# stevenrobertson/cuburn

Hardware: AMD Instinct MI355X
Metric: Msamples/s into 1920x1080 histogram + DE-filter GB/s vs HBM roofline (higher is better)
Workload: dtype f32; 1 GPU; BASELINE configs[1]: 1920x1080 still, 3 xforms (linear+spherical+swirl), 2^28 samples/frame, filters yuv+bilateral+logscale+colorclip, rgba8 out; walker_waves=4, walker_slots=1024, temporal_samples=1024, samples_per_frame=268435456, accum=binned, fuse=256, nslots=1024, frames_queued_ahead=2, frames_per_gpu=1121, parallelism=frame-sharded x1, RCCL gather of device frames, 4 frames per collective

## Files before the change

cuburn_amd/csrc/de.hip:

```cpp
#include "flame_device.h"
#include "kernels.h"
#include "tone_device.h"
#include <utility>
#include <cmath>
#include <algorithm>
#include <cstdlib>
#include <cstring>

struct DeImgPlain {
    float4 *p;
    __device__ __forceinline__ float4 ld(uint32_t i) const { return const_cast<const float4 *>(p)[i]; }
    __device__ __forceinline__ void st(uint32_t i, float4 v) const { p[i] = v; }
};
struct DeCoefs { float k[7]; float k2[19]; };
struct DeSpatial { float s[16]; };

__host__ __device__ constexpr int de_num_x(int P) { constexpr int n[8] = {2, 0, 2, -2, 2, -1, 2, 1}; return n[P]; }
__host__ __device__ constexpr int de_num_y(int P) { constexpr int n[8] = {0, 2, 2, 2, 1, 2, -1, 2}; return n[P]; }
__host__ __device__ constexpr int de_rne_half(int v)
{
    return (v % 2 == 0) ? v / 2 : ((v - 1) / 2 % 2 == 0 ? (v - 1) / 2 : (v + 1) / 2);
}
__host__ __device__ constexpr int de_dx(int P, int r) { return de_rne_half(de_num_x(P) * r); }
__host__ __device__ constexpr int de_dy(int P, int r) { return de_rne_half(de_num_y(P) * r); }
__host__ __device__ constexpr int de_k(int P) { constexpr int k[8] = {0, 0, 2, -2, 4, -1, -4, 1}; return k[P]; }
__host__ __device__ constexpr int de_floor_half(int v) { return v >= 0 ? v / 2 : -((-v + 1) / 2); }
__host__ __device__ constexpr int de_shear(int P, int j) { return de_floor_half(j * de_k(P)); }
__host__ __device__ constexpr int de_dv(int P, int par, int dx, int dy)
{
    return dx - (de_shear(P, par + dy) - de_shear(P, par));
}
__host__ __device__ constexpr bool de_hoisted(int P) { return P < 4; }
constexpr uint32_t DE_RUN = 8u;
struct DeReach { int hu, hv; };
__host__ __device__ constexpr DeReach de_reach(int P, bool blur)
{
    int hu = 0, hv = 0;
    for (int par = 0; par < 2; ++par)
        for (int r = -16; r <= 16; ++r)
            for (int i = -3; i <= 3; ++i)
                for (int j = -3; j <= 3; ++j) {
                    if (!blur && (i != 0 || j != 0 || r == 16 || r == -16)) continue;
                    if ((r == 16 || r == -16) && (i != 0 || j != 0 || de_hoisted(P))) continue;
                    int u = de_dy(P, r), v = de_dv(P, par, de_dx(P, r), de_dy(P, r));
                    int p1 = (par + u) & 1;
                    v += de_dv(P, p1, de_dx(P, 2 * i), de_dy(P, 2 * i)); u += de_dy(P, 2 * i);
                    int p2 = (par + u) & 1;
                    v += de_dv(P, p2, de_dx(P, j), de_dy(P, j)); u += de_dy(P, j);
                    hu = (u < 0 ? -u : u) > hu ? (u < 0 ? -u : u) : hu;
                    hv = (v < 0 ? -v : v) > hv ? (v < 0 ? -v : v) : hv;
                }
    return DeReach{hu, hv};
}

template <int P> struct DeGeo {
    static constexpr int K = de_k(P);
    static constexpr int TW = P == 0 ? 64 : 8;
    static constexpr int TH = P == 0 ? 4 : 32;
    static constexpr int NT = TW * TH;
    static_assert(NT % 64 == 0 && NT <= 1024 && (P == 0 ? TW % 64 == 0 : 64 % TW == 0 && TH % (128 / TW) == 0), "whole waves, rows of equal parity per wave");
    static constexpr bool HOIST = de_hoisted(P);
    static constexpr int HU = de_reach(P, true).hu, HV = de_reach(P, true).hv;
    static constexpr int ROWS = TH + 2 * HU, COLS = TW + 2 * HV, NPX = ROWS * COLS;
    static constexpr bool ROWWISE = P != 0;
    static constexpr int RS = (K & 1) ? (NT / COLS) & ~1 : NT / COLS, NACT = ROWWISE ? RS * COLS : NT;
    static constexpr int NIT = ROWWISE ? (ROWS + RS - 1) / RS : (NPX + NT - 1) / NT;
    static constexpr int HA = de_dy(P, 16) < 0 ? -de_dy(P, 16) : de_dy(P, 16);
    static constexpr int AROWS = TH + 2 * HA, NPXA = AROWS * COLS, AOFF = (HU - HA) * COLS;
    static_assert(HA <= HU, "the taps reach no further than the blurs");
    static constexpr int HBU = de_reach(P, false).hu, HBV = de_reach(P, false).hv;
    static constexpr int BROWS = TH + 2 * HBU, BCOLS = TW + 2 * HBV;
    static constexpr int BPAD = (!de_hoisted(P) && (K & 1) == 0 && TW == 8) ? 12 - BCOLS : 0;
    static constexpr int BSTR = BCOLS + BPAD, NPXB = BROWS * BSTR;
    static_assert(BPAD >= 0 && (BPAD == 0 || (2 * BSTR) % 16 == 8), "rows two apart must lie 8 float4 slots apart mod 16");
    static constexpr int RSB = (K & 1) ? (NT / BCOLS) & ~1 : NT / BCOLS, NACTB = ROWWISE ? RSB * BCOLS : NT;
    static constexpr int NITB = ROWWISE ? (BROWS + RSB - 1) / RSB : (NPXB + NT - 1) / NT;
    static constexpr int MINW = 8;
    static constexpr size_t LDS = (size_t)(NPXA + NPXB) * 16 + (de_hoisted(P) ? (size_t)NPX * 4 : 0) + 64;
    static constexpr int SPAN = de_shear(P, TH - 1) < 0 ? -de_shear(P, TH - 1) : de_shear(P, TH - 1);
    static constexpr int SHMIN = de_shear(P, -HU) < de_shear(P, ROWS - 1 - HU) ? de_shear(P, -HU) : de_shear(P, ROWS - 1 - HU);
    static constexpr int SHMAX = de_shear(P, -HU) < de_shear(P, ROWS - 1 - HU) ? de_shear(P, ROWS - 1 - HU) : de_shear(P, -HU);
    static constexpr int XS = COLS + SHMAX - SHMIN, NF = 2 * ROWS + 2 * XS;
    static_assert((2 * NPX + 2 * NF) * 4 <= NPXB * 16, "preparation planes + frame tables must fit into plane B's space");
    static constexpr int off(int par, int dx, int dy) { return dy * COLS + de_dv(P, par, dx, dy); }
    static constexpr int offb(int par, int dx, int dy) { return dy * BSTR + de_dv(P, par, dx, dy); }
    static constexpr int tap_off(int par, int r) { return off(par, de_dx(P, r), de_dy(P, r)); }
    static constexpr int tap_offb(int par, int r) { return offb(par, de_dx(P, r), de_dy(P, r)); }
    static constexpr int min_tap_off(int par)
    {
        int m = 0;
        for (int r = -16; r <= 16; ++r) m = tap_off(par, r) < m ? tap_off(par, r) : m;
        return m;
    }
    static constexpr int min_tap_offb(int par)
    {
        int m = 0;
        for (int r = -15; r <= 15; ++r) m = tap_offb(par, r) < m ? tap_offb(par, r) : m;
        return m;
    }
};

__device__ __forceinline__ int de_clampi(int v, int lo, int hi) { return min(max(v, lo), hi); }

template <int P, class IMG>
__device__ float de_b1_global(const IMG &N, const fl_dim &d, int cx, int cy, const DeCoefs &k)
{
    float den = 0.0f;
#pragma unroll
    for (int j = 0; j < 7; ++j) {
        const int x = de_clampi(cx + de_dx(P, j - 3), 0, (int)d.astride - 1), y = de_clampi(cy + de_dy(P, j - 3), 0, (int)d.ah - 1);
        den += N.ld((uint32_t)(y * (int)d.astride + x)).w * k.k[j];
    }
    return den;
}
template <int P, class IMG>
__device__ float de_b2_global(const IMG &N, const fl_dim &d, int cx, int cy, const DeCoefs &k)
{
    float den = 0.0f;
#pragma unroll
    for (int i = 0; i < 7; ++i) {
        const int x = de_clampi(cx + de_dx(P, 2 * (i - 3)), 0, (int)d.astride - 1), y = de_clampi(cy + de_dy(P, 2 * (i - 3)), 0, (int)d.ah - 1);
        den += de_b1_global<P>(N, d, x, y, k) * k.k[i];
    }
    return den;
}
template <int P, class IMG>
__device__ float de_b12_global(const IMG &N, const fl_dim &d, int cx, int cy, const DeCoefs &k, float &b1)
{
    float den = 0.0f;
#pragma unroll
    for (int i = 0; i < 7; ++i) {
        const int x = de_clampi(cx + de_dx(P, 2 * (i - 3)), 0, (int)d.astride - 1), y = de_clampi(cy + de_dy(P, 2 * (i - 3)), 0, (int)d.ah - 1);
        const float v = de_b1_global<P>(N, d, x, y, k);
        if (i == 3) b1 = v;
        den += v * k.k[i];
    }
    return den;
}

template <int P>
__device__ __forceinline__ void de_out_px(int wv, int lane, int &ou, int &ov)
{
    using G = DeGeo<P>;
    if (P == 0) { constexpr int WPR = G::TW / 64; ou = wv / WPR; ov = (wv % WPR) * 64 + lane; }
    else if (G::TW == 8 && !G::HOIST) {
        const int q = (lane & 31) >> 2, grp = (q ^ (q >> 1) ^ (q >> 2)) & 1, rank = q >> 1;
        const int gi = 2 * (lane >> 5) + grp;
        const int k = (gi >> 1) * 4 + (gi & 1) + 2 * (rank >> 1);
        ov = ((rank & 1) << 2) | (lane & 3);
        ou = (G::K & 1) ? (wv >> 1) * 16 + (wv & 1) + 2 * k : wv * 8 + k;
    }
    else if (G::K & 1) {
        constexpr int RPW = 64 / G::TW;
        ou = (wv >> 1) * (2 * RPW) + (wv & 1) + 2 * (lane / G::TW); ov = lane % G::TW;
    } else {
        ou = wv * (64 / G::TW) + lane / G::TW; ov = lane % G::TW;
    }
}
__device__ __forceinline__ int de_lane_here()
{
    int l;
    asm volatile("v_mbcnt_lo_u32_b32 %0, -1, 0\n\tv_mbcnt_hi_u32_b32 %0, -1, %0" : "=v"(l));
    return l;
}

typedef float f4v __attribute__((ext_vector_type(4)));
typedef float f2v __attribute__((ext_vector_type(2)));
struct DeTap { f4v a, b; };

#define DE_RD128(dst, addr, boff) asm volatile("ds_read_b128 %0, %1 offset:%2" : "=v"(dst) : "v"(addr), "n"(boff) : "memory")

template <int P> __host__ __device__ constexpr int de_tap_reads(int r)
{
    if (r > 15) return 0;
    return ((r < 15 || !de_hoisted(P)) ? 1 : 0) + (r != 0 ? 1 : 0);

}

template <int P, int PAR, bool SLOW>
__device__ __forceinline__ void de_tap_loop(const float4 *__restrict__ sA, const float4 *__restrict__ sB, int wv,
                                            float cs2, const DeSpatial &spk, float4 &res)
{
    using G = DeGeo<P>;
    int ou, ov;
    de_out_px<P>(wv, de_lane_here(), ou, ov);
    const int ci = (ou + G::HA) * G::COLS + ov + G::HV;
    const int cb = (ou + G::HBU) * G::BSTR + ov + G::HBV;
    constexpr int MINOFF = G::min_tap_off(PAR), MINOFFB = G::min_tap_offb(PAR);
#define TOFF(r) (G::tap_off(PAR, (r)) - MINOFF)
#define TOFFB(r) (G::tap_offb(PAR, (r)) - MINOFFB)
    static_assert((G::tap_off(PAR, 16) - MINOFF) * 16 < 65536 && (G::tap_off(PAR, -16) - MINOFF) >= 0, "tap offsets must fit the DS immediate");
    const float4 *__restrict__ bA = sA + (ci + MINOFF);
    const float4 *__restrict__ bB = sB + (cb + MINOFFB);
    uint32_t aA = (uint32_t)(size_t)bA, aB = (uint32_t)(size_t)bB;
    const float4 cen = bA[TOFF(0)];
    const float cfix = cen.w * frcp(cen.w + 1.0e-6f);
    const float ccx = cen.x * cfix, ccy = cen.y * cfix, ccz = cen.z * cfix;
    const bool cen_live = cen.w > 0.0f;
    float cs2h = cs2;
    asm volatile("" : "+s"(cs2h));
    const float m2u = -2.0f * cs2h;
    const float m2 = cen_live ? m2u : 0.0f;
    float Cx = ccx * m2, Cy = ccy * m2, Cz = ccz * m2;
    const float Kp = 0.5f * cs2;
    float Dl = cen_live ? cs2 * fmaf(ccz, ccz, fmaf(ccy, ccy, ccx * ccx)) - Kp : 0.0f;
    float dcs = cen_live ? 0.0f : cs2;
    const float y0c = fmaf(cs2, fmaf(cen.z, cen.z, fmaf(cen.y, cen.y, cen.x * cen.x)), Kp) + Dl;
    float cds = bB[TOFFB(0)].x;
    float wprev = G::HOIST ? 0.0f : bA[TOFF(-16)].w;
    const float4 p0 = bA[TOFF(-15)];
    f4v pix = {p0.x, p0.y, p0.z, p0.w};
    f2v oxy = {0.0f, 0.0f}, ozw = {0.0f, 0.0f};
    float wsum = 0.0f;

    constexpr int NBUF = SLOW ? 1 : 2;
    DeTap L[NBUF][2];
    auto issue = [&](auto gc) __attribute__((always_inline)) {
        constexpr int g = decltype(gc)::value;
#define ISSUE_TAP(k) if constexpr (-15 + g * 2 + (k) <= 15) { \
            constexpr int r = -15 + g * 2 + (k); \
            if constexpr (r < 15 || !G::HOIST) DE_RD128(L[g % NBUF][k].a, aA, TOFF(r + 1) * 16); \
            if constexpr (r != 0) DE_RD128(L[g % NBUF][k].b, aB, TOFFB(r) * 16); }
        ISSUE_TAP(0) ISSUE_TAP(1)
#undef ISSUE_TAP
    };
    auto step = [&](auto gc) __attribute__((always_inline)) {
        constexpr int g = decltype(gc)::value;
        if constexpr (SLOW) issue(gc);
        else if constexpr (g + 1 < 16) issue(std::integral_constant<int, g + 1>{});
        constexpr int inflight = (!SLOW && g + 1 < 16) ? de_tap_reads<P>(-15 + (g + 1) * 2) + de_tap_reads<P>(-14 + (g + 1) * 2) : 0;
        DeTap (&T)[2] = L[g % NBUF];
#define DE_WAIT_OPS "+v"(T[0].a), "+v"(T[0].b), "+v"(T[1].a), "+v"(T[1].b), "+v"(aA), "+v"(aB), "+v"(oxy), "+v"(ozw), "+v"(wsum), \
                    "+v"(pix), "+v"(wprev), "+v"(Cx), "+v"(Cy), "+v"(Cz), "+v"(Dl), "+v"(cds)
        if constexpr (SLOW) asm volatile("s_waitcnt lgkmcnt(%[n])" : DE_WAIT_OPS, "+v"(dcs) : [n] "n"(inflight));
        else asm volatile("s_waitcnt lgkmcnt(%[n])" : DE_WAIT_OPS : [n] "n"(inflight));
#undef DE_WAIT_OPS
        constexpr int r0 = -15 + g * 2, r1 = r0 + 1;
        constexpr bool two = r1 <= 15;
        const f4v px0 = pix, px1 = T[0].a;
        f4v b0 = T[0].b, b1 = T[1].b;
        float t0, t1 = 0.0f;
        if constexpr (r0 == 0) t0 = SLOW ? fmaf(cs2, fmaf(px0.z, px0.z, fmaf(px0.y, px0.y, px0.x * px0.x)), 0.5f * cs2) + Dl : y0c;
        else t0 = fmaf(b0.y, Dl, G::HOIST ? (r0 < 0 ? b0.w : b0.z) : b0.z);
        if constexpr (two) {
            if constexpr (r1 == 0) t1 = SLOW ? fmaf(cs2, fmaf(px1.z, px1.z, fmaf(px1.y, px1.y, px1.x * px1.x)), 0.5f * cs2) + Dl : y0c;
            else t1 = fmaf(b1.y, Dl, G::HOIST ? (r1 < 0 ? b1.w : b1.z) : b1.z);
        }
        t0 = fmaf(px0.z, Cz, t0); if constexpr (two) t1 = fmaf(px1.z, Cz, t1);
        t0 = fmaf(px0.y, Cy, t0); if constexpr (two) t1 = fmaf(px1.y, Cy, t1);
        t0 = fmaf(px0.x, Cx, t0); if constexpr (two) t1 = fmaf(px1.x, Cx, t1);
        if constexpr (SLOW) {
            if constexpr (r0 != 0) t0 = fmaf(fmaf(px0.z, px0.z, fmaf(px0.y, px0.y, px0.x * px0.x)), -dcs, t0);
            if constexpr (two && r1 != 0) t1 = fmaf(fmaf(px1.z, px1.z, fmaf(px1.y, px1.y, px1.x * px1.x)), -dcs, t1);
        }
        float e0 = t0, e1 = t1;
        if constexpr (r0 != 0) { const float d0 = cds - b0.x; e0 = t0 - fabsf(d0); }
        if constexpr (two && r1 != 0) { const float d1 = cds - b1.x; e1 = t1 - fabsf(d1); }
        if constexpr (!G::HOIST) {
            float g0 = 0.0f, g1 = 0.0f;
            if constexpr (r0 != 0) g0 = (T[0].a.w - wprev) * b0.w;
            if constexpr (two && r1 != 0) g1 = (T[1].a.w - px0.w) * b1.w;
            if constexpr (r0 != 0) g0 = fexp2(r0 < 0 ? -g0 : g0);
            if constexpr (two && r1 != 0) g1 = fexp2(r1 < 0 ? -g1 : g1);
            if constexpr (r0 != 0) e0 -= g0;
            if constexpr (two && r1 != 0) e1 -= g1;
        }
        float f0 = fexp2(e0), f1 = two ? fexp2(e1) : 0.0f;
        f0 *= spk.s[r0 < 0 ? -r0 : r0]; if constexpr (two) f1 *= spk.s[r1 < 0 ? -r1 : r1];
        const float fw0 = f0 * px0.w, fw1 = f1 * px1.w;
        wsum += f0;
        oxy.x = fmaf(fw0, px0.x, oxy.x); oxy.y = fmaf(fw0, px0.y, oxy.y); ozw.x = fmaf(fw0, px0.z, ozw.x); ozw.y += fw0;
        if constexpr (two) {
            wsum += f1;
            oxy.x = fmaf(fw1, px1.x, oxy.x); oxy.y = fmaf(fw1, px1.y, oxy.y); ozw.x = fmaf(fw1, px1.z, ozw.x); ozw.y += fw1;
            wprev = px1.w;
            if (r1 < 15 || !G::HOIST) pix = T[1].a;
        }
    };
    if constexpr (!SLOW) issue(std::integral_constant<int, 0>{});
    [&]<int... Gs>(std::integer_sequence<int, Gs...>) __attribute__((always_inline)) {
        (step(std::integral_constant<int, Gs>{}), ...);
    }(std::make_integer_sequence<int, 16>{});
#undef TOFF
#undef TOFFB
    const float ow = ozw.y;
    const float wn = ow * frcp(wsum + 1e-10f);
    const float rn = ow >= 1.17549435e-38f ? frcp(ow) : 0.0f;
    res = make_float4(oxy.x * rn, oxy.y * rn, ozw.x * rn, wn);
}

template <int P, int PAR>
__device__ __forceinline__ void de_tap_loop_slow(const float4 *__restrict__ sA, const float4 *__restrict__ sB, int wv,
                                              float cs2, const DeSpatial &spk, float4 &res)
{
    de_tap_loop<P, PAR, true>(sA, sB, wv, cs2, spk, res);
}

__device__ __forceinline__ float4 de_yuv_px(float4 p)
{
    const float u = p.y - 0.5f * p.w, v = p.z - 0.5f * p.w;
    return make_float4(fmaxf(0.0f, p.x + 1.402f * v), fmaxf(0.0f, p.x - 0.34414f * u - 0.71414f * v), fmaxf(0.0f, p.x + 1.772f * u), p.w);
}
template <int IN>
__device__ __forceinline__ float4 de_in_px(float4 p)
{
    if (IN == 0) return p;
    if (IN == 2) p = de_yuv_px(p);
    const float rw = p.w > 0.0f ? frcp(p.w) : 0.0f;
    return make_float4(p.x * rw, p.y * rw, p.z * rw, p.w);
}

#define DE_IN_PX(p) de_in_px<IN>(p)
template <int P, int IN, int OUT>
__global__ void __launch_bounds__(DeGeo<P>::NT, DeGeo<P>::MINW)
k_de_dir(fl_dim d, float4 *__restrict__ Nout_, const float4 *__restrict__ N_, DeCoefs kc, DeSpatial spk,
         float cs2, float ads, float dpow, float gspeed, uint32_t tiles_y, uint32_t ntiles, uint32_t tiles_x, uint32_t magic, DeTail tail)
{
    using G = DeGeo<P>;
    static_assert(2 * G::NPX * 4 <= G::NPXB * 16, "the preparation planes must fit into plane B's space");
    extern __shared__ __attribute__((aligned(16))) unsigned char smem[];
    float4 *sA = reinterpret_cast<float4 *>(smem);
    float4 *sB = reinterpret_cast<float4 *>(smem + (size_t)G::NPXA * 16);
    float *sW = reinterpret_cast<float *>(sB);
    float *s1 = sW + G::NPX;
    float *sF1 = s1 + G::NPX, *sF2 = sF1 + G::NF;
    float *sWf = reinterpret_cast<float *>(smem + (size_t)(G::NPXA + G::NPXB) * 16);
    const DeImgPlain N = {const_cast<float4 *>(N_)}, Nout = {Nout_};

    const uint32_t per_xcd = (ntiles + 7u) / 8u, xcd = blockIdx.x & 7u;
    int tx, ty;
    if (tail.order == 0) {
        const uint32_t t = xcd * per_xcd + (xcd < 4u ? (blockIdx.x >> 3) : per_xcd - 1u - (blockIdx.x >> 3));
        if (t >= ntiles) return;
        const uint32_t q = tiles_y == 1u ? t : __umulhi(t, magic);
        tx = (int)q; ty = (int)(t - q * tiles_y);
    } else {
        const uint32_t loc = blockIdx.x >> 3;
        const uint32_t rm = tail.order == 1 ? blockIdx.x : ((loc / DE_RUN) * 8u + xcd) * DE_RUN + loc % DE_RUN;
        if (rm >= ntiles) return;
        const uint32_t q = tiles_x == 1u ? rm : __umulhi(rm, magic);
        ty = (int)q; tx = (int)(rm - q * tiles_x);
        ty = ty == 0 ? (int)tiles_y - 1 : ty - 1;
    }
    const int bx0 = tx * G::TW - (G::K > 0 ? G::SPAN : 0), by0 = ty * G::TH;
    const int tid = threadIdx.x;
    const int xmax = (int)d.astride - 1, ymax = (int)d.ah - 1;
    const bool border = by0 - G::HU < 0 || by0 + G::TH + G::HU > (int)d.ah ||
                        bx0 + min(0, de_shear(P, -G::HU)) + min(0, de_shear(P, G::TH + G::HU)) - G::HV - 1 < 0 ||
                        bx0 + max(0, de_shear(P, -G::HU)) + max(0, de_shear(P, G::TH + G::HU)) + G::TW + G::HV + 1 > (int)d.astride;

#define DE_S_THREAD() int ts_ = tid; asm volatile("" : "+v"(ts_)); \
    const int sr0 = G::ROWWISE ? ts_ / G::COLS : 0, sc0 = ts_ - sr0 * G::COLS; const bool sact = ts_ < G::NACT; \
     \
    auto s_elem = [&](int it, int &idx, int &ul, int &vl) __attribute__((always_inline)) -> bool { \
        idx = it * G::NACT + tid; \
        if (G::ROWWISE) { ul = it * G::RS + sr0; vl = sc0; return sact && ul < G::ROWS; } \
        ul = idx / G::COLS; vl = idx - ul * G::COLS; return idx < G::NPX; }; \
     \
    auto s_elem_clamped = [&](int it, int &ul, int &vl) __attribute__((always_inline)) { \
        if (G::ROWWISE) { ul = min(it * G::RS + sr0, G::ROWS - 1); vl = sc0; } \
        else { const int idx = min(it * G::NT + tid, G::NPX - 1); ul = idx / G::COLS; vl = idx - ul * G::COLS; } }
#define DE_B_THREAD() int tb_ = tid; asm volatile("" : "+v"(tb_)); \
    const int br0 = G::ROWWISE ? tb_ / G::BCOLS : 0, bc0 = tb_ - br0 * G::BCOLS; const bool bact = tb_ < G::NACTB; \
    const int bidx0 = (br0 + G::HU - G::HBU) * G::COLS + bc0 + G::HV - G::HBV;       \
    const int bsto0 = br0 * G::BSTR + bc0;                                           \
     \
    auto b_elem = [&](int it, int &bidx, int &idx, int &ul, int &vl) __attribute__((always_inline)) -> bool { \
        if (G::ROWWISE) { const int ub = it * G::RSB + br0; ul = ub + G::HU - G::HBU; vl = bc0 + G::HV - G::HBV; \
                          bidx = bsto0 + it * G::RSB * G::BSTR; \
                          idx = bidx0 + it * G::RSB * G::COLS; return bact && ub < G::BROWS; } \
        static_assert(G::ROWWISE || G::BSTR == G::BCOLS, "padding only with row-wise staging"); \
        bidx = it * G::NACTB + tid; \
        const int ub = bidx / G::BCOLS, vb = bidx - ub * G::BCOLS; \
        ul = ub + G::HU - G::HBU; vl = vb + G::HV - G::HBV; idx = ul * G::COLS + vl; return bidx < G::NPXB; }

    __builtin_amdgcn_s_setprio(3);
#ifdef DE_X_TAPSONLY
    if (gspeed != 12345.0f) goto taps;
#endif
#ifdef DE_X_STOP_AFTER
#define DE_X_STOP(n) if (DE_X_STOP_AFTER == n && gspeed != 12345.0f) { if (tid == 0 && sB[17].x == 1.2345e-33f) Nout.st(0, sB[17]); return; }
#else
#define DE_X_STOP(n)
#endif
    if (G::HOIST && !border) {
        float4 tq[G::NIT];
        DE_S_THREAD();
#pragma unroll
        for (int it = 0; it < G::NIT; ++it) {
            int ul, vl;
            s_elem_clamped(it, ul, vl);
            const int gx = bx0 + (((ul - G::HU) * G::K) >> 1) + vl - G::HV, gy = by0 + ul - G::HU;
            tq[it] = DE_IN_PX(N.ld((uint32_t)(gy * (int)d.astride + gx)));
        }
#pragma unroll
        for (int it = 0; it < G::NIT; ++it) {
            int idx, ul, vl;
            if (s_elem(it, idx, ul, vl)) {
                sWf[idx] = tq[it].w;
                if (idx >= G::AOFF && idx < G::AOFF + G::NPXA) sA[idx - G::AOFF] = tq[it];
            }
        }
        __syncthreads();
        DE_X_STOP(1)
        DE_B_THREAD();
#pragma unroll
        for (int it = 0; it < G::NITB; ++it) {
            int bidx, idx, ul, vl;
            if (!b_elem(it, bidx, idx, ul, vl)) continue;
            float den = 0.0f;
#pragma unroll
            for (int m = -9; m <= 9; ++m) den = fmaf(sWf[idx + G::off(0, de_dx(P, m), de_dy(P, m))], kc.k2[m + 9], den);
            const float ra = frcp(den + 1.0e-6f) * gspeed;
            const float4 n = sA[idx - G::AOFF];
            constexpr int dn = G::off(0, de_dx(P, 1), de_dy(P, 1));
            const float g = (sWf[idx + dn] - sWf[idx - dn]) * ra;
            const float yk = fmaf(cs2, fmaf(n.z, n.z, fmaf(n.y, n.y, n.x * n.x)), 0.5f * cs2);
            sB[bidx] = make_float4(ads * de_pow(n.w, dpow), n.w > 0.0f ? 1.0f : 0.0f, yk - fexp2(g), yk - fexp2(-g));
        }
        __syncthreads();
        DE_X_STOP(4)
    } else {
    float4 tn[G::NIT];
    {
    DE_S_THREAD();
    if (G::ROWWISE && !border) {
        const int u0 = sr0 - G::HU;
        const uint32_t g0 = (uint32_t)((by0 + u0) * (int)d.astride + bx0 + ((u0 * G::K) >> 1) + sc0 - G::HV);
        const uint32_t gstep = (uint32_t)(G::RS * (int)d.astride + G::RS * G::K / 2);
#pragma unroll
        for (int it = 0; it < G::NIT; ++it) {
            const int nrows = G::ROWS - it * G::RS < G::RS ? G::ROWS - it * G::RS : G::RS;
            if (sr0 < nrows) tn[it] = DE_IN_PX(N.ld(g0 + (uint32_t)it * gstep));
            else tn[it] = make_float4(0.0f, 0.0f, 0.0f, 0.0f);
        }
    } else {
#pragma unroll
    for (int it = 0; it < G::NIT; ++it) {
        int ul, vl;
        s_elem_clamped(it, ul, vl);
        const int gx = de_clampi(bx0 + (((ul - G::HU) * G::K) >> 1) + vl - G::HV, 0, xmax);
        const int gy = de_clampi(by0 + ul - G::HU, 0, ymax);
        tn[it] = DE_IN_PX(N.ld((uint32_t)(gy * (int)d.astride + gx)));
    }
    }
    if (border) {
        const int x0a = bx0 - G::HV, nrows_top = min(G::ROWS, G::HU - by0), first_bot = max(0, ymax + 1 - (by0 - G::HU));
        int tlo = 1, thi = 0, blo = 1, bhi = 0;
        if (nrows_top > 0) {
            const int a = x0a + de_shear(P, -G::HU), b = x0a + (((nrows_top - 1 - G::HU) * G::K) >> 1);
            tlo = min(a, b); thi = max(a, b) + G::COLS - 1;
        }
        if (first_bot < G::ROWS) {
            const int a = x0a + (((first_bot - G::HU) * G::K) >> 1), b = x0a + de_shear(P, G::ROWS - 1 - G::HU);
            blo = min(a, b); bhi = max(a, b) + G::COLS - 1;
        }
        for (int e = tid; e < G::NF; e += G::NT) {
            int fx, fy; bool need;
            if (e < 2 * G::ROWS) {
                const int side = e >= G::ROWS, u = e - side * G::ROWS;
                const int x0 = x0a + (((u - G::HU) * G::K) >> 1);
                need = side ? x0 + G::COLS - 1 > xmax : x0 < 0;
                fx = side ? xmax : 0; fy = de_clampi(by0 + u - G::HU, 0, ymax);
            } else {
                const int e2 = e - 2 * G::ROWS, side = e2 >= G::XS;
                fx = x0a + G::SHMIN + e2 - side * G::XS; fy = side ? ymax : 0;
                need = fx >= 0 && fx <= xmax && (side ? (fx >= blo && fx <= bhi) : (fx >= tlo && fx <= thi));
            }
            if (need) {
                float b1;
                sF2[e] = de_b12_global<P>(N, d, fx, fy, kc, b1);
                sF1[e] = b1;
            }
        }
    }
#pragma unroll
    for (int it = 0; it < G::NIT; ++it) {
        int idx, ul, vl;
        if (s_elem(it, idx, ul, vl)) {
            sW[idx] = tn[it].w;
            if (idx >= G::AOFF && idx < G::AOFF + G::NPXA) sA[idx - G::AOFF] = tn[it];
        }
    }
    }
    __syncthreads();
    DE_X_STOP(1)

    {
    DE_S_THREAD();
#pragma unroll
    for (int it = 0; it < G::NIT; ++it) {
        int idx, ul, vl;
        if (!s_elem(it, idx, ul, vl)) continue;
        const bool par = ((ul - G::HU) & 1) != 0;
        float den = 0.0f;
#pragma unroll
        for (int j = 0; j < 7; ++j) {
            const int o0 = G::off(0, de_dx(P, j - 3), de_dy(P, j - 3)), o1 = G::off(1, de_dx(P, j - 3), de_dy(P, j - 3));
            const int o = (G::K & 1) ? (par ? o1 : o0) : o0;
            den = fmaf(sW[idx + o], kc.k[j], den);
        }
        if (border) {
            const int gxu = bx0 + (((ul - G::HU) * G::K) >> 1) + vl - G::HV, gyu = by0 + ul - G::HU;
            if (gxu < 0 || gxu > xmax || gyu < 0 || gyu > ymax)
                den = sF1[gxu < 0 ? ul : gxu > xmax ? G::ROWS + ul : 2 * G::ROWS + (gyu < 0 ? 0 : G::XS) + gxu - (bx0 - G::HV + G::SHMIN)];
        }
        s1[idx] = den;
    }
    }
    __syncthreads();
    DE_X_STOP(2)

    float4 pb[G::NITB];
    {
    DE_B_THREAD();
#pragma unroll
    for (int it = 0; it < G::NITB; ++it) {
        pb[it] = make_float4(0.0f, 0.0f, 0.0f, 0.0f);
        int bidx, idx, ul, vl;
        if (!b_elem(it, bidx, idx, ul, vl)) continue;
        const bool par = ((ul - G::HU) & 1) != 0;
        float den = 0.0f;
#pragma unroll
        for (int i = 0; i < 7; ++i) {
            const int o0 = G::off(0, de_dx(P, 2 * (i - 3)), de_dy(P, 2 * (i - 3))), o1 = G::off(1, de_dx(P, 2 * (i - 3)), de_dy(P, 2 * (i - 3)));
            const int o = (G::K & 1) ? (par ? o1 : o0) : o0;
            den = fmaf(s1[idx + o], kc.k[i], den);
        }
        if (border) {
            const int gxu = bx0 + (((ul - G::HU) * G::K) >> 1) + vl - G::HV, gyu = by0 + ul - G::HU;
            if (gxu < 0 || gxu > xmax || gyu < 0 || gyu > ymax)
                den = sF2[gxu < 0 ? ul : gxu > xmax ? G::ROWS + ul : 2 * G::ROWS + (gyu < 0 ? 0 : G::XS) + gxu - (bx0 - G::HV + G::SHMIN)];
        }
        const float ra = frcp(den + 1.0e-6f) * gspeed;
        const float4 n = sA[idx - G::AOFF];
        pb[it].x = ads * de_pow(n.w, dpow);
        pb[it].y = n.w > 0.0f ? 1.0f : 0.0f;
        const float yk = fmaf(cs2, fmaf(n.z, n.z, fmaf(n.y, n.y, n.x * n.x)), 0.5f * cs2);
        if (G::HOIST) {
            constexpr int dn = G::off(0, de_dx(P, 1), de_dy(P, 1));
            const float g = (sW[idx + dn] - sW[idx - dn]) * ra;
            pb[it].z = yk - fexp2(g);
            pb[it].w = yk - fexp2(-g);
        } else {
            pb[it].z = yk;
            pb[it].w = ra;
        }
    }
    }
    __syncthreads();
    DE_X_STOP(3)
    {
    DE_B_THREAD();
#pragma unroll
    for (int it = 0; it < G::NITB; ++it) {
        int bidx, idx, ul, vl;
        if (b_elem(it, bidx, idx, ul, vl)) sB[bidx] = pb[it];
    }
    }
    __syncthreads();
    DE_X_STOP(4)

    }
#ifdef DE_X_TAPSONLY
taps:
#endif
    __builtin_amdgcn_s_setprio(0);
    const int wv = __builtin_amdgcn_readfirstlane(tid >> 6);
    do {
    float4 res;
    {
        int cu, cv;
        de_out_px<P>(wv, tid & 63, cu, cv);
        {
            const int xq = bx0 + ((cu * G::K) >> 1) + cv, yq = by0 + cu;
            if (__builtin_amdgcn_ballot_w64(xq >= 0 && xq <= xmax && yq <= ymax) == 0ull) continue;
        }
        const bool slow = __builtin_amdgcn_ballot_w64(!(sA[(cu + G::HA) * G::COLS + cv + G::HV].w > 0.0f)) != 0ull;
        if ((G::K & 1) && (wv & 1)) { if (slow) de_tap_loop_slow<P, 1>(sA, sB, wv, cs2, spk, res); else de_tap_loop<P, 1, false>(sA, sB, wv, cs2, spk, res); }
        else { if (slow) de_tap_loop_slow<P, 0>(sA, sB, wv, cs2, spk, res); else de_tap_loop<P, 0, false>(sA, sB, wv, cs2, spk, res); }
    }
    int ou, ov;
    de_out_px<P>(wv, de_lane_here(), ou, ov);

    const int xo = bx0 + ((ou * G::K) >> 1) + ov, yo = by0 + ou;
    if (xo >= 0 && xo <= xmax && yo <= ymax) {
        if (OUT) {
            float4 p = make_float4(res.x * res.w, res.y * res.w, res.z * res.w, res.w);
            if (tail.do_log) p = logscale_px(p, tail.k1, tail.k2);
            if (tail.do_clip) p = colorclip_px(p, tail.vib, tail.highpow, tail.gam, tail.lin, tail.lingam);
            res = p;
        }
        Nout.st((uint32_t)(yo * (int)d.astride + xo), res);
    }
    } while (false);
}

template <int P, int IN, int OUT>
static void launch_de_dir_one(hipStream_t st, fl_dim d, float4 *Nout, const float4 *N, DeCoefs kc, DeSpatial spk,
                              float cs2, float ads, float dpow, float gspeed, DeTail tail)
{
    using G = DeGeo<P>;
    static_assert(G::LDS * (G::MINW * 256 / G::NT) <= 160 * 1024, "LDS must allow MINW waves per SIMD");
    static unsigned long long attr = 0;
    ensure_max_dynamic_lds((const void *)k_de_dir<P, IN, OUT>, attr);
    const uint32_t tiles_x = (d.astride + G::SPAN + G::TW - 1) / G::TW, tiles_y = (d.ah + G::TH - 1) / G::TH;
    const uint32_t ntiles = tiles_x * tiles_y;
    const uint32_t gran = tail.order == 2 ? 8u * DE_RUN : 8u;
    const uint32_t divisor = tail.order == 0 ? tiles_y : tiles_x, magic = (uint32_t)(0x100000000ull / divisor) + 1u;
    if ((unsigned long long)(ntiles + gran) * divisor >= 0x100000000ull) abort();
    hipLaunchKernelGGL((k_de_dir<P, IN, OUT>), dim3(gran * ((ntiles + gran - 1) / gran)), dim3(G::NT), G::LDS, st, d, Nout, N, kc, spk,
                       cs2, ads, dpow, gspeed, tiles_y, ntiles, tiles_x, magic, tail);
}

void launch_de_dir(hipStream_t st, fl_dim d, int pattern, float4 *Nout, const float4 *N, const float *coefs7,
                   float sstd, float cstd, float dstd, float dpow, float gspeed, int in_mode, const DeTail *tail)
{
    DeCoefs kc;
    for (int i = 0; i < 7; ++i) kc.k[i] = coefs7[i];
    for (int m = -9; m <= 9; ++m) {
        float a = 0.0f;
        for (int i = -3; i <= 3; ++i) { const int j = m - 2 * i; if (j >= -3 && j <= 3) a += coefs7[i + 3] * coefs7[j + 3]; }
        kc.k2[m + 9] = a;
    }
    DeSpatial spk;
    for (int r = 0; r < 16; ++r) spk.s[r] = expf((float)(r * r) / (-1.41421353816986f * sstd));
    const float cs2 = 1.0f / (-1.41421353816986f * 3.0f * cstd) * 1.44269502162933f;
    const float ads = fabsf(-0.5f / dstd);
    DeTail none = {};
    static const char *forced_s = getenv("FLAME_DE_ORDER");
    const int forced = !forced_s || !*forced_s ? -1 : (strlen(forced_s) == 8 ? forced_s[pattern] - '0' : forced_s[0] - '0');
    const bool beyond_mall = (size_t)d.astride * d.ah * 16u > ((size_t)256 << 20);
    const int table = (pattern == 1) ? 0 : (pattern == 5 || pattern == 7) ? (beyond_mall ? 2 : 0) : 2;
    const int order = forced >= 0 && forced <= 2 ? forced : table;
    none.order = order;
    DeTail tl = tail ? *tail : none;
    tl.order = order;
#define DE(P, I, O) launch_de_dir_one<P, I, O>(st, d, Nout, N, kc, spk, cs2, ads, dpow, gspeed, tl)
    switch (pattern) {
    case 0:
        if (in_mode == 2) DE(0, 2, 0); else if (in_mode == 1) DE(0, 1, 0); else abort();
        break;
    case 1: DE(1, 0, 0); break;
    case 2: DE(2, 0, 0); break;
    case 3: DE(3, 0, 0); break;
    case 4: DE(4, 0, 0); break;
    case 5: DE(5, 0, 0); break;
    case 6: DE(6, 0, 0); break;
    case 7: DE(7, 0, 1); break;
    default: break;
    }
#undef DE
}
```

cuburn_amd/csrc/flame_abi.hip:

```cpp
#include <hip/hip_runtime.h>
#include <cstdio>
#include <cstdlib>
#include <cstring>
#include <cmath>
#include <string>
#include <atomic>
#include <vector>
#include <algorithm>
#include "kernels.h"
#include "flame_device.h"

static thread_local std::string g_err;
static int fail(int code, const char *what, const char *file, int line, hipError_t e = hipSuccess)
{
    char buf[512];
    if (e != hipSuccess) snprintf(buf, sizeof buf, "%s: %s (%s:%d)", what, hipGetErrorString(e), file, line);
    else snprintf(buf, sizeof buf, "%s (%s:%d)", what, file, line);
    g_err = buf;
    return code;
}
#define HIPCHK(x) do { hipError_t e_ = (x); if (e_ != hipSuccess) \
    return fail(e_ == hipErrorOutOfMemory ? FL_E_NOMEM : FL_E_HIP, #x, __FILE__, __LINE__, e_); } while (0)
#define REQUIRE(c, msg) do { if (!(c)) return fail(FL_E_INVAL, msg, __FILE__, __LINE__); } while (0)

struct EvPair { hipEvent_t a, b; };

struct Lane {
    hipStream_t stream = nullptr;
    size_t nbins = 0;
    float4 *d_front = nullptr, *d_back = nullptr, *d_side = nullptr;
    float *d_blur = nullptr;
    u64 *d_atom = nullptr;
    uint32_t *d_hot = nullptr;
    void *d_outpix = nullptr;
    uint32_t *d_de_tmax = nullptr;
    float *d_de_sinv = nullptr;
    size_t outpix_bytes = 0;
    uint32_t *d_log[2] = {nullptr, nullptr}, *d_dir[2] = {nullptr, nullptr};
    size_t log_words[2] = {0, 0}, dir_words[2] = {0, 0};
    hipStream_t aux = nullptr;
    hipEvent_t ev_it[2] = {nullptr, nullptr}, ev_ac[2] = {nullptr, nullptr};
    float *d_params = nullptr;
    uint64_t params_serial = 0;
    size_t params_floats = 0;
    u64 *d_palette = nullptr;
    hipEvent_t ev_interp_done = nullptr;
    hipEvent_t ev_iter_done = nullptr;
    hipEvent_t ev_out_done = nullptr;
    bool interp_rec = false, iter_rec = false, out_rec = false;
    bool pend_yuv = false, pend_finish = false, pend_log = false;
    float pend_k1 = 0.0f, pend_k2 = 0.0f;
    int pend_in_mode = 0;
    float pend_dp[5] = {0, 0, 0, 0, 0}, pend_k7[7] = {0, 0, 0, 0, 0, 0, 0};
    fl_dim pend_dim = {0, 0, 0, 0, 0};
};

struct fl_ctx {
    int device = 0;
    bool own_stream = false;
    static const int kMaxLanes = 4;
    int nlanes = 2, cur = 0;
    Lane lanes[kMaxLanes];
    uint32_t nslots = 0, nwalkers = 0;
    uint32_t sub_log2 = 0;
    uint32_t ntemporal() const { return nslots << sub_log2; }
    int nw = 4;
    fl_mwc *d_rng = nullptr;
    float4 *d_points = nullptr;
    u64 *d_counters = nullptr;
    uint32_t *d_sort = nullptr; size_t sort_words = 0;
    uint32_t bin_rounds = 16, bin_parts = 0;
    uint32_t launch_rounds = 0;
    uint32_t round_counter = 0;
    static const uint32_t kFrames = 8;
    hipEvent_t ev_begin_[kFrames] = {}, ev_end_[kFrames] = {};
    uint32_t frame_lane[kFrames] = {};
    uint32_t frame_seq = 0;
    std::vector<EvPair> pool, iter_ev, accum_ev, flush_ev, filt_ev, de_ev;
    size_t pool_used = 0;
    bool timing = true;
    static const uint32_t kDepEvents = 16;
    hipEvent_t dep_ev[kDepEvents] = {};
    uint32_t dep_next = 0;
    bool env_bin_wide = false, env_no_intra = false;
    bool use_rtc = true;
    uint32_t n_spec_launch = 0, n_interp_launch = 0;
};
#define L(c) ((c)->lanes[(c)->cur])
#define OTHER(c) ((c)->lanes[((c)->cur + (c)->nlanes - 1) % (c)->nlanes])
#define FL_NOUT 65536u

struct fl_genome {
    uint64_t serial = 0;
    std::vector<int32_t> prog;
    IterSpec spec;
    hipFunction_t rtc_fn[5][2][4] = {};
    unsigned rtc_epoch = 0;
    bool rtc_failed = false;
    uint32_t nops = 0, nrows = 0, pstride = 0;
    int32_t *d_prog = nullptr, *d_ops = nullptr;
    float *d_times = nullptr, *d_knots = nullptr, *d_ptimes = nullptr;
    float4 *d_pals = nullptr;
    uint32_t npal = 0;
    static const int kStage = 4;
    unsigned char *h_stage[kStage] = {};
    hipEvent_t ev_stage[kStage] = {};
    size_t stage_bytes = 0;
    int stage_next = 0;
};

static const int kKnownVars[] = {0,1,2,3,4,5,6,7,8,9,10,11,12,13,14,15,16,17,18,19,20,21,22,23,24,25,26,27,28,29,30,31,32,33,
    34,35,36,37,38,39,40,41,42,43,44,45,46,48,49,50,51,52,53,54,55,56,57,58,59,60,61,62,63,64,65,66,67,68,69,70,71,72,73,
    74,75,76,77,80,81,82,83,84,85,86,87,88,89,90,91,92,93,94,95,97,98};

static const size_t kMaxTimed = 8192;

static EvPair *ev_begin(fl_ctx *c, std::vector<EvPair> &list)
{
    if (!c->timing || c->pool_used >= kMaxTimed) return nullptr;
    if (c->pool.capacity() < kMaxTimed) c->pool.reserve(kMaxTimed);
    if (c->pool_used == c->pool.size()) {
        EvPair p;
        if (hipEventCreate(&p.a) != hipSuccess || hipEventCreate(&p.b) != hipSuccess) return nullptr;
        c->pool.push_back(p);
    }
    EvPair p = c->pool[c->pool_used++];
    list.push_back(p);
    hipEventRecord(p.a, L(c).stream);
    return &c->pool[c->pool_used - 1];
}
static EvPair *ev_pair(fl_ctx *c, std::vector<EvPair> &list)
{
    if (!c->timing || c->pool_used >= kMaxTimed) return nullptr;
    if (c->pool.capacity() < kMaxTimed) c->pool.reserve(kMaxTimed);
    if (c->pool_used == c->pool.size()) {
        EvPair p;
        if (hipEventCreate(&p.a) != hipSuccess || hipEventCreate(&p.b) != hipSuccess) return nullptr;
        c->pool.push_back(p);
    }
    list.push_back(c->pool[c->pool_used++]);
    return &c->pool[c->pool_used - 1];
}
static void ev_end(fl_ctx *c, EvPair *p) { if (p) hipEventRecord(p->b, L(c).stream); }
static EvPair *ev_begin_on(fl_ctx *c, std::vector<EvPair> &list, hipStream_t st)
{
    EvPair *p = ev_pair(c, list);
    if (p) hipEventRecord(p->a, st);
    return p;
}
static void ev_end_on(EvPair *p, hipStream_t st) { if (p) hipEventRecord(p->b, st); }

#pragma GCC visibility push(default)
extern "C" {

int fl_abi_version(void) { return FL_ABI_VERSION; }
const char *fl_last_error(void) { return g_err.c_str(); }

void fl_calc_dim(uint32_t w, uint32_t h, fl_dim *o)
{
    o->w = w; o->h = h;
    o->aw = w + 2 * FL_GUTTER;
    o->ah = 16 * ((h + 2 * FL_GUTTER + 15) / 16);
    o->astride = 32 * ((o->aw + 31) / 32);
}

static void flush_pending(fl_ctx *c);

static const float *de_norms()
{
    static const std::vector<float> t = [] { std::vector<float> v(16 * FL_DE_MAX_RADIUS + 1); de_adaptive_norms(v.data()); return v; }();
    return t.data();
}

static void free_fb(fl_ctx *c)
{
    hipFree(L(c).d_front); hipFree(L(c).d_back); hipFree(L(c).d_side); hipFree(L(c).d_blur);
    hipFree(L(c).d_atom); hipFree(L(c).d_hot); hipFree(L(c).d_outpix); hipFree(L(c).d_de_tmax); hipFree(L(c).d_de_sinv);
    L(c).d_front = L(c).d_back = L(c).d_side = nullptr; L(c).d_blur = nullptr; L(c).d_atom = nullptr;
    L(c).d_hot = nullptr; L(c).d_outpix = nullptr; L(c).d_de_tmax = nullptr; L(c).d_de_sinv = nullptr;
    L(c).nbins = 0; L(c).outpix_bytes = 0;
    L(c).pend_yuv = L(c).pend_finish = L(c).pend_log = false;
}

static int ensure_fb(fl_ctx *c, const fl_dim &d)
{
    size_t nbins = (size_t)d.ah * d.astride, ob = (size_t)d.w * d.h * 8;
    if (L(c).nbins >= nbins && L(c).outpix_bytes >= ob) return FL_OK;
    hipStreamSynchronize(L(c).stream);
    free_fb(c);
    hipError_t e;
    if ((e = hipMalloc(&L(c).d_front, 16 * nbins)) || (e = hipMalloc(&L(c).d_back, 16 * nbins)) ||
        (e = hipMalloc(&L(c).d_side, 16 * nbins)) || (e = hipMalloc(&L(c).d_blur, 4 * nbins)) ||
        (e = hipMalloc(&L(c).d_atom, 8 * nbins)) || (e = hipMalloc(&L(c).d_hot, 4 * (nbins / 16))) ||
        (e = hipMalloc(&L(c).d_outpix, ob)) ||
        (e = hipMalloc(&L(c).d_de_tmax, 4 * (nbins / 256 + 64))) ||
        (e = hipMalloc(&L(c).d_de_sinv, 4 * (16 * FL_DE_MAX_RADIUS + 1))) ||
        (e = hipMemcpyAsync(L(c).d_de_sinv, de_norms(), 4 * (16 * FL_DE_MAX_RADIUS + 1), hipMemcpyHostToDevice, L(c).stream))) {
        free_fb(c);
        (void)hipGetLastError();
        return fail(e == hipErrorOutOfMemory ? FL_E_NOMEM : FL_E_HIP, "framebuffer allocation", __FILE__, __LINE__, e);
    }
    L(c).nbins = nbins; L(c).outpix_bytes = ob;
    return FL_OK;
}

static bool env_on(const char *name) { const char *e = getenv(name); return e && *e && strcmp(e, "0") != 0; }

int fl_ctx_create(int device, void *stream, const fl_mwc *seeds, uint32_t nseeds, uint32_t nslots, fl_ctx **out)
{
    REQUIRE(out && seeds, "null argument");
    REQUIRE((nslots >= FL_NTEMPORAL || nslots == FL_NTEMPORAL / 2 || nslots == FL_NTEMPORAL / 4) && nslots % 256 == 0 && nslots <= 16384,
            "nslots must be a multiple of 256 in [1024, 16384] (or 512 slots of 8 waves / 256 of 16: two / four temporal samples per workgroup)");
    int ndev = 0;
    if (hipGetDeviceCount(&ndev) != hipSuccess || ndev <= 0) return fail(FL_E_NODEV, "no HIP device", __FILE__, __LINE__);
    REQUIRE(device >= 0 && device < ndev, "bad device index");
    HIPCHK(hipSetDevice(device));
    hipDeviceProp_t prop;
    HIPCHK(hipGetDeviceProperties(&prop, device));
    if (strncmp(prop.gcnArchName, "gfx950", 6) != 0)
        return fail(FL_E_NODEV, "device is not gfx950 (kernels are built for MI355X only)", __FILE__, __LINE__);
    int nw = 0;
    {
        const uint32_t fixed = FL_PAL_H * 256 + FL_NOUT;
        const uint32_t per_wave = nslots * 64u;
        if (nseeds == fixed + 16u * per_wave) nw = 16;
        else if (nseeds == fixed + 8u * per_wave) nw = 8;
        else if (nseeds == fixed + 4u * per_wave) nw = 4;
        else return fail(FL_E_INVAL, "nseeds must be nslots*64*NW + 64*256 + 65536 with NW = 4, 8 or 16", __FILE__, __LINE__);
    }
    fl_ctx *c = new fl_ctx;
    c->device = device;
    c->nw = nw;
    if (nslots < FL_NTEMPORAL && (uint32_t)nw * nslots != 4u * FL_NTEMPORAL)
        return fail(FL_E_INVAL, "512 slots need 8-wave workgroups, 256 slots 16-wave ones (a temporal sample per four waves: 1024 in all)", __FILE__, __LINE__);
    c->nslots = nslots;
    c->sub_log2 = nslots >= FL_NTEMPORAL ? 0u : nw == 8 ? 1u : 2u;
    c->nwalkers = nslots * (uint32_t)nw * 64 + FL_PAL_H * 256 + FL_NOUT;
    if (const char *e = getenv("FLAME_LANES")) { const int v = atoi(e); c->nlanes = v >= 1 && v <= fl_ctx::kMaxLanes ? v : 2; }
    if (const char *e = getenv("FLAME_BIN_ROUNDS")) { int v = atoi(e); if (v >= 1 && v <= FL_BIN_R_MAX) c->bin_rounds = (uint32_t)v; }
    if (const char *e = getenv("FLAME_BIN_PARTS")) { int v = atoi(e); if (v >= 1 && v <= 64) c->bin_parts = (uint32_t)v; }
    c->env_bin_wide = env_on("FLAME_BIN_WIDE");
    if (const char *e = getenv("FLAME_RTC")) c->use_rtc = strcmp(e, "0") != 0;
    c->env_no_intra = env_on("FLAME_NO_INTRA_OVERLAP");
    if (const char *e = getenv("FLAME_LAUNCH_ROUNDS")) { int v = atoi(e); if (v >= 16 && v <= 4096) c->launch_rounds = (uint32_t)(v / 16 * 16); }
    if (stream) { c->lanes[0].stream = (hipStream_t)stream; c->own_stream = false; c->nlanes = 1; }
    else c->own_stream = true;
    hipError_t e = hipSuccess;
    const char *what = "context allocation";
    do {
        if (c->own_stream)
            for (int i = 0; i < c->nlanes && e == hipSuccess; ++i) e = hipStreamCreateWithFlags(&c->lanes[i].stream, hipStreamNonBlocking);
        if (e) break;
        if ((e = hipMalloc(&c->d_rng, sizeof(fl_mwc) * (size_t)c->nwalkers))) break;
        if ((e = hipMalloc(&c->d_points, sizeof(float4) * (size_t)nslots * nw * 64))) break;
        if ((e = hipMalloc(&c->d_counters, 8 * 4))) break;
        for (int i = 0; i < c->nlanes && e == hipSuccess; ++i) {
            Lane &ln = c->lanes[i];
            if ((e = hipMalloc(&ln.d_palette, sizeof(u64) * FL_PAL_H * FL_PAL_W))) break;
            if ((e = hipEventCreateWithFlags(&ln.ev_interp_done, hipEventDisableTiming))) break;
            if ((e = hipEventCreateWithFlags(&ln.ev_iter_done, hipEventDisableTiming))) break;
            if ((e = hipEventCreateWithFlags(&ln.ev_out_done, hipEventDisableTiming))) break;
            if ((e = hipStreamCreateWithFlags(&ln.aux, hipStreamNonBlocking))) break;
            for (int k = 0; k < 2 && e == hipSuccess; ++k) {
                if ((e = hipEventCreateWithFlags(&ln.ev_it[k], hipEventDisableTiming))) break;
                e = hipEventCreateWithFlags(&ln.ev_ac[k], hipEventDisableTiming);
            }
            if (e) break;
        }
        if (e) break;
        if ((e = hipMemcpy(c->d_rng, seeds, sizeof(fl_mwc) * (size_t)c->nwalkers, hipMemcpyHostToDevice))) break;
        if ((e = hipMemsetD32(c->d_points, 0x7fc00000, (size_t)nslots * nw * 64 * 4))) break;
        if ((e = hipMemset(c->d_counters, 0, 32))) break;
        for (uint32_t i = 0; i < fl_ctx::kFrames && e == hipSuccess; ++i) {
            if ((e = hipEventCreate(&c->ev_begin_[i]))) break;
            e = hipEventCreate(&c->ev_end_[i]);
        }
    } while (0);
    if (e != hipSuccess) {
        fl_ctx_destroy(c);
        (void)hipGetLastError();
        return fail(e == hipErrorOutOfMemory ? FL_E_NOMEM : FL_E_HIP, what, __FILE__, __LINE__, e);
    }
    *out = c;
    return FL_OK;
}

static void sync_all(fl_ctx *c)
{
    for (int i = 0; i < c->nlanes; ++i) { hipStreamSynchronize(c->lanes[i].stream); if (c->lanes[i].aux) hipStreamSynchronize(c->lanes[i].aux); }
}

void fl_ctx_destroy(fl_ctx *c)
{
    if (!c) return;
    hipSetDevice(c->device);
    for (uint32_t i = 0; i < fl_ctx::kDepEvents; ++i) if (c->dep_ev[i]) hipEventDestroy(c->dep_ev[i]);
    for (int i = 0; i < fl_ctx::kMaxLanes; ++i) {
        if (c->lanes[i].stream) hipStreamSynchronize(c->lanes[i].stream);
        if (c->lanes[i].aux) hipStreamSynchronize(c->lanes[i].aux);
    }
    for (int i = 0; i < fl_ctx::kMaxLanes; ++i) {
        c->cur = i;
        free_fb(c);
        Lane &ln = c->lanes[i];
        hipFree(ln.d_params); hipFree(ln.d_palette);
        for (int k = 0; k < 2; ++k) {
            hipFree(ln.d_log[k]); hipFree(ln.d_dir[k]);
            if (ln.ev_it[k]) hipEventDestroy(ln.ev_it[k]);
            if (ln.ev_ac[k]) hipEventDestroy(ln.ev_ac[k]);
        }
        if (ln.aux) hipStreamDestroy(ln.aux);
        if (ln.ev_interp_done) hipEventDestroy(ln.ev_interp_done);
        if (ln.ev_iter_done) hipEventDestroy(ln.ev_iter_done);
        if (ln.ev_out_done) hipEventDestroy(ln.ev_out_done);
        if (c->own_stream && ln.stream) hipStreamDestroy(ln.stream);
    }
    hipFree(c->d_rng); hipFree(c->d_points); hipFree(c->d_counters); hipFree(c->d_sort);
    for (auto &p : c->pool) { hipEventDestroy(p.a); hipEventDestroy(p.b); }
    for (uint32_t i = 0; i < fl_ctx::kFrames; ++i) {
        if (c->ev_begin_[i]) hipEventDestroy(c->ev_begin_[i]);
        if (c->ev_end_[i]) hipEventDestroy(c->ev_end_[i]);
    }
    (void)hipGetLastError();
    delete c;
}

int fl_ctx_sync(fl_ctx *c) { REQUIRE(c, "null ctx"); sync_all(c); return FL_OK; }

static int wait_other(fl_ctx *c, int what)
{
    if (c->nlanes < 2) return FL_OK;
    Lane &o = OTHER(c);
    if (what == 0 && o.interp_rec) HIPCHK(hipStreamWaitEvent(L(c).stream, o.ev_interp_done, 0));
    if (what == 1 && o.iter_rec) HIPCHK(hipStreamWaitEvent(L(c).stream, o.ev_iter_done, 0));
    if (what == 2 && o.out_rec) HIPCHK(hipStreamWaitEvent(L(c).stream, o.ev_out_done, 0));
    return FL_OK;
}

static int check_prog(const int32_t *p, uint32_t n)
{
    REQUIRE(n >= FL_PROG_HDR && p[0] == FL_PROG_MAGIC, "bad program header");
    int nxf = p[1], hf = p[2], ps = p[3], cdf = p[4], xo = p[5], xs = p[6], vs = p[7];
    REQUIRE(nxf >= 1 && nxf <= FL_MAX_XFORMS && (hf == 0 || hf == 1), "bad xform count");
    REQUIRE(ps >= 6 + nxf && ps <= FL_MAX_PSTRIDE, "bad pstride");
    REQUIRE(cdf >= 6 && cdf + nxf <= xo, "bad cdf offset");
    REQUIRE(xs >= FL_XF_HDR + vs && (xs % 4) == 0 && vs >= 2 && vs <= 64, "bad record strides");
    REQUIRE(xo + (nxf + hf) * xs <= ps, "xform records exceed the block");
    return FL_OK;
}

static bool known_var(int id)
{
    for (int k : kKnownVars) if (k == id) return true;
    return false;
}

int fl_genome_create(fl_ctx *c, const int32_t *prog, uint32_t nprog, const int32_t *ops, uint32_t nops,
                     uint32_t nrows, fl_genome **out)
{
    REQUIRE(c && prog && ops && out, "null argument");
    int rc = check_prog(prog, nprog);
    if (rc) return rc;
    REQUIRE(nrows >= 1 && nrows <= 4096 && nops >= 1, "bad row / op count");
    uint32_t ps = prog[3];
    const int xo = prog[5], xs = prog[6], vs = prog[7], nrec = prog[1] + prog[2];
    std::vector<int> nvar_seen(nrec, -1), opac_seen(nrec, 0), opac_ops(nrec, 0);
    for (uint32_t i = 0; i < nops; ++i) {
        const int32_t *o = ops + 4 * i;
        REQUIRE(o[0] >= FL_OP_SPLINE && o[0] <= FL_OP_OPACITY, "bad op kind");
        REQUIRE(o[1] >= 0 && (uint32_t)o[1] < ps, "op destination out of range");
        if (o[0] != FL_OP_CONST) {
            uint32_t ndst = 1, nsrc = 1;
            switch (o[0]) {
            case FL_OP_CAMERA: ndst = 6; nsrc = 4; break;
            case FL_OP_AFFINE: ndst = 6; nsrc = 6; break;
            case FL_OP_CDF:
                REQUIRE(o[3] >= 1 && o[3] <= FL_MAX_XFORMS, "bad CDF length");
                ndst = nsrc = (uint32_t)o[3];
                break;
            case FL_OP_PERSP: ndst = 3; break;
            default: break;
            }
            REQUIRE((uint32_t)o[1] + ndst <= ps, "op destination out of range");
            REQUIRE(o[2] >= 0 && (uint32_t)o[2] + nsrc <= nrows, "op row out of range");
            if (o[0] == FL_OP_RATIO2 || o[0] == FL_OP_PERSP) REQUIRE(o[3] >= 0 && (uint32_t)o[3] < nrows, "op row out of range");
            if (o[0] == FL_OP_OPACITY) {
                const int rel = o[1] - xo;
                REQUIRE(rel >= 0 && rel / xs < prog[1] && rel % xs == 15, "opacity op must write word 15 of a selectable xform record");
                ++opac_ops[rel / xs];
            }
            continue;
        }
        const int rel = o[1] - xo;
        REQUIRE(rel >= 0 && rel / xs < nrec, "structure word outside the xform records");
        const int w = rel % xs;
        if (w == 14) {
            const int nv = o[2] & 0xff;
            REQUIRE(FL_XF_HDR + nv * vs <= xs && (o[2] >> 10) == 0, "bad variation count");
            REQUIRE(((o[2] >> 9) & 1) == 0 || rel / xs < prog[1], "the final xform has no opacity");
            nvar_seen[rel / xs] = nv;
            opac_seen[rel / xs] = (o[2] >> 9) & 1;
        } else {
            REQUIRE(w >= FL_XF_HDR && (w - FL_XF_HDR) % vs == 0, "misplaced structure word");
            if (!known_var(o[2])) return fail(FL_E_UNSUPPORTED, "unknown variation id", __FILE__, __LINE__);
        }
    }
    for (int i = 0; i < nrec; ++i) REQUIRE(nvar_seen[i] >= 0, "xform record without a variation count");
    for (int i = 0; i < nrec; ++i) REQUIRE(opac_ops[i] == opac_seen[i], "opacity flag and opacity op do not match");
    IterSpec spec;
    spec.nxf = prog[1]; spec.has_final = prog[2]; spec.pstride = prog[3]; spec.cdf_off = prog[4];
    spec.xf_off = xo; spec.xf_stride = xs; spec.var_stride = vs;
    spec.nvar.assign(nrec, 0); spec.post.assign(nrec, 0); spec.opac.assign(nrec, 0); spec.vids.assign(nrec, std::vector<int>());
    for (int i = 0; i < nrec; ++i) spec.vids[i].assign(nvar_seen[i], -1);
    for (uint32_t i = 0; i < nops; ++i) {
        const int32_t *o = ops + 4 * i;
        if (o[0] != FL_OP_CONST) continue;
        const int rel = o[1] - xo, rec = rel / xs, w = rel % xs;
        if (w == 14) { spec.nvar[rec] = o[2] & 0xff; spec.post[rec] = (o[2] >> 8) & 1; spec.opac[rec] = (o[2] >> 9) & 1; }
        else {
            const int j = (w - FL_XF_HDR) / vs;
            if (j < (int)spec.vids[rec].size()) spec.vids[rec][j] = o[2];
        }
    }
    for (int i = 0; i < nrec; ++i)
        for (int v : spec.vids[i]) REQUIRE(v >= 0, "variation record without a variation number");
    HIPCHK(hipSetDevice(c->device));
    fl_genome *g = new fl_genome;
    { static std::atomic<uint64_t> next_serial{1}; g->serial = next_serial.fetch_add(1); }
    g->spec = spec;
    g->prog.assign(prog, prog + nprog);
    g->nops = nops; g->nrows = nrows; g->pstride = ps;
    g->stage_bytes = 2 * 4 * (size_t)nrows * FL_KNOTS + 16 * 256 * (FL_KNOTS - 1) + 4 * FL_KNOTS;
    hipError_t e = hipSuccess;
    do {
        if ((e = hipMalloc(&g->d_prog, 4 * nprog))) break;
        if ((e = hipMalloc(&g->d_ops, 16 * nops))) break;
        if ((e = hipMalloc(&g->d_times, 4 * (size_t)nrows * FL_KNOTS))) break;
        if ((e = hipMalloc(&g->d_knots, 4 * (size_t)nrows * FL_KNOTS))) break;
        if ((e = hipMalloc(&g->d_ptimes, 4 * FL_KNOTS))) break;
        if ((e = hipMalloc(&g->d_pals, 16 * 256 * FL_KNOTS))) break;
        if ((e = hipMemcpy(g->d_prog, prog, 4 * nprog, hipMemcpyHostToDevice))) break;
        if ((e = hipMemcpy(g->d_ops, ops, 16 * nops, hipMemcpyHostToDevice))) break;
        if ((e = hipMemset(g->d_pals, 0, 16 * 256 * FL_KNOTS))) break;
        for (int i = 0; i < fl_genome::kStage && e == hipSuccess; ++i) {
            if ((e = hipHostMalloc((void **)&g->h_stage[i], g->stage_bytes, hipHostMallocDefault))) break;
            e = hipEventCreateWithFlags(&g->ev_stage[i], hipEventDisableTiming);
        }
    } while (0);
    if (e != hipSuccess) {
        fl_genome_destroy(g);
        (void)hipGetLastError();
        return fail(e == hipErrorOutOfMemory ? FL_E_NOMEM : FL_E_HIP, "genome allocation", __FILE__, __LINE__, e);
    }
    *out = g;
    return FL_OK;
}

void fl_genome_destroy(fl_genome *g)
{
    if (!g) return;
    hipFree(g->d_prog); hipFree(g->d_ops); hipFree(g->d_times); hipFree(g->d_knots);
    hipFree(g->d_ptimes); hipFree(g->d_pals);
    for (int i = 0; i < fl_genome::kStage; ++i) { if (g->h_stage[i]) hipHostFree(g->h_stage[i]); if (g->ev_stage[i]) hipEventDestroy(g->ev_stage[i]); }
    delete g;
}

int fl_genome_upload(fl_ctx *c, fl_genome *g, const float *times, const float *knots,
                     const float *pal_rgba, const float *pal_times, uint32_t npal)
{
    REQUIRE(c && g && times && knots && pal_rgba && pal_times, "null argument");
    REQUIRE(npal >= 1 && npal < FL_KNOTS, "bad palette count");
    HIPCHK(hipSetDevice(c->device));
    const size_t nb = 4 * (size_t)g->nrows * FL_KNOTS, pb = 16 * 256 * (size_t)npal, tb = 4 * FL_KNOTS;
    const int slot = g->stage_next;
    g->stage_next = (slot + 1) % fl_genome::kStage;
    HIPCHK(hipEventSynchronize(g->ev_stage[slot]));
    unsigned char *h = g->h_stage[slot];
    memcpy(h, times, nb);
    memcpy(h + nb, knots, nb);
    memcpy(h + 2 * nb, pal_rgba, pb);
    memcpy(h + 2 * nb + pb, pal_times, tb);
    { int rc = wait_other(c, 0); if (rc) return rc; }
    HIPCHK(hipMemcpyAsync(g->d_times, h, nb, hipMemcpyHostToDevice, L(c).stream));
    HIPCHK(hipMemcpyAsync(g->d_knots, h + nb, nb, hipMemcpyHostToDevice, L(c).stream));
    HIPCHK(hipMemcpyAsync(g->d_pals, h + 2 * nb, pb, hipMemcpyHostToDevice, L(c).stream));
    HIPCHK(hipMemcpyAsync(g->d_ptimes, h + 2 * nb + pb, tb, hipMemcpyHostToDevice, L(c).stream));
    HIPCHK(hipEventRecord(g->ev_stage[slot], L(c).stream));
    g->npal = npal;
    return FL_OK;
}

int fl_frame_begin(fl_ctx *c, uint32_t *frame_id)
{
    REQUIRE(c && frame_id, "null argument");
    HIPCHK(hipSetDevice(c->device));
    const uint32_t id = c->frame_seq++;
    const uint32_t k = id % fl_ctx::kFrames;
    c->cur = (int)(id % (uint32_t)c->nlanes);
    c->frame_lane[k] = (uint32_t)c->cur;
    HIPCHK(hipEventRecord(c->ev_begin_[k], L(c).stream));
    HIPCHK(hipEventRecord(c->ev_end_[k], L(c).stream));
    *frame_id = id;
    return FL_OK;
}

int fl_interp(fl_ctx *c, fl_genome *g, uint32_t w, uint32_t h, float ts, float td)
{
    REQUIRE(c && g && g->npal, "genome not uploaded");
    HIPCHK(hipSetDevice(c->device));
    fl_dim d; fl_calc_dim(w, h, &d);
    const size_t need = (size_t)c->ntemporal() * g->pstride;
    if (need > L(c).params_floats) {
        HIPCHK(hipStreamSynchronize(L(c).stream));
        hipFree(L(c).d_params); L(c).d_params = nullptr; L(c).params_floats = 0;
        HIPCHK(hipMalloc(&L(c).d_params, sizeof(float) * need));
        L(c).params_floats = need; L(c).params_serial = 0;
    }
    fl_mwc *rng_pal = c->d_rng + (size_t)c->nslots * c->nw * 64;
    { int rc = wait_other(c, 0); if (rc) return rc; }
    launch_interp_palette(L(c).stream, rng_pal, g->d_ptimes, g->d_pals, ts, td / FL_PAL_H, L(c).d_palette);
    launch_interp_params(L(c).stream, L(c).d_params, g->d_times, g->d_knots, g->d_ops, g->nops, g->pstride,
                         c->ntemporal(), ts, td / (float)c->ntemporal(), d, L(c).params_serial != g->serial);
    L(c).params_serial = g->serial;
    HIPCHK(hipGetLastError());
    HIPCHK(hipEventRecord(L(c).ev_interp_done, L(c).stream));
    L(c).interp_rec = true;
    return FL_OK;
}

static int do_clear(fl_ctx *c, const fl_dim &d, bool reset_points)
{
    size_t nbins = (size_t)d.ah * d.astride;
    launch_clear_frame(L(c).stream, L(c).d_front, L(c).d_atom, L(c).d_hot, c->d_counters, c->d_points, (uint32_t)nbins,
                       reset_points ? c->nslots * (uint32_t)c->nw * 64u : 0u);
    HIPCHK(hipGetLastError());
    return FL_OK;
}

#define FL_BIN_MAX_ROUNDS 1024u
#define FL_BIN_MAX_ROUNDS_LONG 2304u

static int ensure_binned(fl_ctx *c, const fl_dim &d, uint32_t write_rounds, int buf, uint32_t *tiles_x, uint32_t *nbins,
                         uint32_t *nbatch_total, bool *wide)
{
    const uint32_t nt = (uint32_t)c->nw * 64;
    const uint32_t rows = (d.ah + FL_TILE_H - 1) / FL_TILE_H;
    *wide = ((d.astride + 127) / 128) * rows > FL_MAX_BINS || c->env_bin_wide;
    const uint32_t tw = *wide ? (1u << FL_TILE_W_WIDE_LOG2) : 128u;
    *tiles_x = (d.astride + tw - 1) / tw;
    *nbins = *tiles_x * rows;
    if (*nbins > FL_MAX_BINS_WIDE) return fail(FL_E_UNSUPPORTED, "image too large for the binned accumulate (> 8191 tiles of 256x64)", __FILE__, __LINE__);
    const uint32_t per_slot = (write_rounds + c->bin_rounds - 1) / c->bin_rounds;
    *nbatch_total = per_slot * c->nslots;
    const size_t region = !*wide && FL_LOG_PACK3 ? 2 * (size_t)fl_pack3_words(c->bin_rounds * nt) : (size_t)c->bin_rounds * nt;
    size_t lw = (size_t)*nbatch_total * region + 8, dw = (size_t)*nbins * *nbatch_total;
    if (lw > L(c).log_words[buf]) {
        HIPCHK(hipStreamSynchronize(L(c).stream)); HIPCHK(hipStreamSynchronize(L(c).aux));
        hipFree(L(c).d_log[buf]); L(c).d_log[buf] = nullptr; L(c).log_words[buf] = 0;
        HIPCHK(hipMalloc(&L(c).d_log[buf], lw * 4));
        L(c).log_words[buf] = lw;
    }
    if (dw > L(c).dir_words[buf]) {
        HIPCHK(hipStreamSynchronize(L(c).stream)); HIPCHK(hipStreamSynchronize(L(c).aux));
        hipFree(L(c).d_dir[buf]); L(c).d_dir[buf] = nullptr; L(c).dir_words[buf] = 0;
        HIPCHK(hipMalloc(&L(c).d_dir[buf], dw * 4));
        L(c).dir_words[buf] = dw;
    }
    return FL_OK;
}

static int do_iter_launch(fl_ctx *c, fl_genome *g, const fl_dim &d, uint32_t nrounds, uint32_t fuse, bool count, int acc = 0,
                          int buf = 0, hipStream_t drain = nullptr)
{
    if (!drain) drain = L(c).stream;
    uint32_t tiles_x = 0, nbins = 0, nbatch_total = 0;
    bool wide = false;
    if (acc == FL_ACCUM_BINNED) {
        if (nrounds <= fuse) return fail(FL_E_INVAL, "binned launch needs write-enabled rounds", __FILE__, __LINE__);
        int rc = ensure_binned(c, d, nrounds - fuse, buf, &tiles_x, &nbins, &nbatch_total, &wide);
        if (rc) return rc;
    }
    EvPair *e = ev_pair(c, c->iter_ev);
    const int kacc = acc == FL_ACCUM_BINNED && wide ? 3 : acc;
    hipFunction_t fn = nullptr;
    if (c->use_rtc && !g->rtc_failed && kacc != 2) {
        const unsigned ep = rtc_epoch();
        if (g->rtc_epoch != ep) { memset(g->rtc_fn, 0, sizeof g->rtc_fn); g->rtc_epoch = ep; }
        hipFunction_t &slot = g->rtc_fn[c->sub_log2 ? 2 + c->sub_log2 : c->nw == 16 ? 2 : c->nw == 8][count ? 1 : 0][kacc];
        if (!slot) {
            std::string err;
            if (rtc_iter_kernel(c->device, g->spec, c->nw, c->nslots, count, kacc, &slot, &err, c->sub_log2)) {
                g->rtc_failed = true;
                slot = nullptr;
                fprintf(stderr, "libflame_hip: per-genome kernel not available (%s); using the interpreter kernel\n", err.c_str());
            }
        }
        fn = slot;
    }
    (fn ? c->n_spec_launch : c->n_interp_launch) += 1;
    if (fn)
        launch_iter_fn(L(c).stream, fn, c->nw, kacc, c->nslots, g->d_prog, L(c).d_params, L(c).d_palette, c->d_rng, c->d_points,
                       L(c).d_hot, L(c).d_atom, (float *)L(c).d_front, c->d_counters, d.astride, d.ah, c->round_counter, nrounds, fuse,
                       tiles_x, nbins, c->bin_rounds, nbatch_total, L(c).d_log[buf], L(c).d_dir[buf],
                       e ? e->a : nullptr, e ? e->b : nullptr, c->sub_log2);
    else
    launch_iter(L(c).stream, c->nw, count, kacc, c->nslots, g->d_prog, L(c).d_params, L(c).d_palette, c->d_rng, c->d_points,
                L(c).d_hot, L(c).d_atom, (float *)L(c).d_front, c->d_counters, d.astride, d.ah, c->round_counter, nrounds, fuse,
                tiles_x, nbins, c->bin_rounds, nbatch_total, L(c).d_log[buf], L(c).d_dir[buf],
                e ? e->a : nullptr, e ? e->b : nullptr, c->sub_log2);
    c->round_counter += nrounds;
    HIPCHK(hipGetLastError());
    if (acc == FL_ACCUM_BINNED) {
        if (drain != L(c).stream) {
            HIPCHK(hipEventRecord(L(c).ev_it[buf], L(c).stream));
            HIPCHK(hipStreamWaitEvent(drain, L(c).ev_it[buf], 0));
        }
        EvPair *e2 = ev_begin_on(c, c->accum_ev, drain);
        uint32_t parts = c->bin_parts ? c->bin_parts : nbins > 512u ? ((wide ? 12800u : 6400u) + nbins / 2u) / nbins : (wide ? 16384u : 8192u) / nbins;
        parts = parts < 1u ? 1u : parts > (c->bin_parts ? 64u : 16u) ? (c->bin_parts ? 64u : 16u) : parts;
        launch_accum_tiles(drain, L(c).d_log[buf], L(c).d_dir[buf], L(c).d_palette, L(c).d_atom, (float *)L(c).d_front, tiles_x, nbins,
                           parts, nbatch_total, c->bin_rounds * (uint32_t)c->nw * 64, c->nslots, d.astride, d.ah, wide);
        ev_end_on(e2, drain);
        HIPCHK(hipGetLastError());
    }
    return FL_OK;
}

static int do_flush(fl_ctx *c, const fl_dim &d, bool use_hot = true, hipStream_t st = nullptr)
{
    if (!st) st = L(c).stream;
    EvPair *e = ev_begin_on(c, c->flush_ev, st);
    launch_flush(st, L(c).d_atom, L(c).d_front, L(c).d_hot, d.ah * d.astride, use_hot);
    ev_end_on(e, st);
    HIPCHK(hipGetLastError());
    return FL_OK;
}

int fl_iterate(fl_ctx *c, fl_genome *g, uint32_t w, uint32_t h, double nsamples, uint32_t fuse,
               int accum_mode, uint64_t *nsamples_run)
{
    REQUIRE(c && g, "null argument");
    REQUIRE(accum_mode == FL_ACCUM_ATOMIC || accum_mode == FL_ACCUM_BINNED || accum_mode == 2, "bad accumulation mode");
    REQUIRE(L(c).params_floats >= (size_t)c->ntemporal() * g->pstride, "fl_interp has not run for this genome");
    HIPCHK(hipSetDevice(c->device));
    fl_dim d; fl_calc_dim(w, h, &d);
    int rc = ensure_fb(c, d);
    if (rc) return rc;
    flush_pending(c);
    if ((rc = wait_other(c, 1))) return rc;
    if ((rc = do_clear(c, d, true))) return rc;
    const uint32_t nt = (uint32_t)c->nw * 64;
    const double per_round = (double)c->nslots * nt;
    uint64_t rounds = (uint64_t)ceil(nsamples / per_round);
    if (rounds == 0) rounds = 1;
    if (nsamples_run) *nsamples_run = (uint64_t)(rounds * per_round);
    const uint64_t unit = 256ull << c->sub_log2;
    auto launches_with = [rounds, unit](uint64_t cap_) { uint32_t nl = 0; for (uint64_t r = rounds, b = 4; r; b += b / 2) { r -= std::min(std::min(r, b * unit), cap_); ++nl; } return nl; };
    const uint64_t cap_short = (uint64_t)FL_BIN_MAX_ROUNDS << c->sub_log2;
    uint64_t cap_long = (uint64_t)(c->nw == 16 ? 1536u : FL_BIN_MAX_ROUNDS_LONG) << c->sub_log2;
    if (accum_mode == FL_ACCUM_BINNED && !c->launch_rounds && launches_with(cap_long) < launches_with(cap_short)) {
        const uint32_t nt_ = (uint32_t)c->nw * 64;
        const bool wide_ = ((d.astride + 127) / 128) * ((d.ah + FL_TILE_H - 1) / FL_TILE_H) > FL_MAX_BINS || c->env_bin_wide;
        const uint32_t tw_ = wide_ ? (1u << FL_TILE_W_WIDE_LOG2) : 128u;
        const size_t nbins_ = (size_t)((d.astride + tw_ - 1) / tw_) * ((d.ah + FL_TILE_H - 1) / FL_TILE_H);
        const size_t region = !wide_ && FL_LOG_PACK3 ? 2 * (size_t)fl_pack3_words(c->bin_rounds * nt_) : (size_t)c->bin_rounds * nt_;
        const size_t nb_long = (size_t)((std::min(rounds, cap_long) + c->bin_rounds - 1) / c->bin_rounds) * c->nslots;
        const size_t need = (nb_long * region + 8 + nbins_ * nb_long) * 4;
        size_t have = 0, grow = 0;
        for (int b = 0; b < 2; ++b) {
            have = (L(c).log_words[b] + L(c).dir_words[b]) * 4;
            if (need > have) grow += need - have;
        }
        size_t mfree = 0, mtotal = 0;
        if (grow && (hipMemGetInfo(&mfree, &mtotal) != hipSuccess || grow + (size_t(1) << 30) > mfree)) cap_long = cap_short;
    }
    const uint64_t cap = accum_mode != FL_ACCUM_BINNED ? ~0ull : c->launch_rounds ? c->launch_rounds :
                         launches_with(cap_long) < launches_with(cap_short) ? cap_long : cap_short;
    const uint32_t nlaunch = launches_with(cap);
    const bool pipelined = accum_mode == FL_ACCUM_BINNED && nlaunch > 1 && !c->env_no_intra;
    hipStream_t drain = pipelined ? L(c).aux : L(c).stream;
    uint64_t batch = 4;
    uint32_t k = 0;
    while (rounds) {
        const uint64_t n = std::min(std::min(rounds, batch * unit), cap);
        const uint32_t f = k == 0 ? fuse : 0;
        const int buf = pipelined ? (int)(k & 1u) : 0;
        if (pipelined && k >= 2) HIPCHK(hipStreamWaitEvent(L(c).stream, L(c).ev_ac[buf], 0));
        if ((rc = do_iter_launch(c, g, d, (uint32_t)n + f, f, false, accum_mode, buf, drain))) return rc;
        if ((rc = do_flush(c, d, accum_mode != FL_ACCUM_BINNED, drain))) return rc;
        if (pipelined) HIPCHK(hipEventRecord(L(c).ev_ac[buf], drain));
        rounds -= n;
        batch += batch / 2;
        ++k;
    }
    HIPCHK(hipEventRecord(L(c).ev_iter_done, L(c).stream));
    L(c).iter_rec = true;
    if (pipelined) {
        HIPCHK(hipStreamWaitEvent(L(c).stream, L(c).ev_ac[(k - 1) & 1u], 0));
        if (k >= 2) HIPCHK(hipStreamWaitEvent(L(c).stream, L(c).ev_ac[k & 1u], 0));
    }
    return FL_OK;
}

static void gauss7(float stdev, float *c)
{
    float s = 0.0f;
    for (int i = 0; i < 7; ++i) { float x = (float)(i - 3); c[i] = expf(x * x / (-2.0f * stdev * stdev)); s += c[i]; }
    for (int i = 0; i < 7; ++i) c[i] /= s;
}

static void run_de_finish(fl_ctx *c, const float *clip)
{
    Lane &ln = L(c);
    DeTail t = {ln.pend_log ? 1 : 0, ln.pend_k1, ln.pend_k2, clip ? 1 : 0, clip ? clip[0] : 0.f, clip ? clip[1] : 0.f,
                clip ? clip[2] : 0.f, clip ? clip[3] : 0.f, clip ? clip[4] : 0.f};
    EvPair *e = ev_begin(c, c->de_ev);
    float4 *Na = ln.d_back, *Nb = ln.d_front;
    launch_de_dir(ln.stream, ln.pend_dim, 0, Na, Nb, ln.pend_k7, ln.pend_dp[0], ln.pend_dp[1], ln.pend_dp[2], ln.pend_dp[3], ln.pend_dp[4], ln.pend_in_mode, nullptr);
    for (int pat = 1; pat < 7; ++pat) {
        launch_de_dir(ln.stream, ln.pend_dim, pat, Nb, Na, ln.pend_k7, ln.pend_dp[0], ln.pend_dp[1], ln.pend_dp[2], ln.pend_dp[3], ln.pend_dp[4]);
        std::swap(Na, Nb);
    }
    launch_de_dir(ln.stream, ln.pend_dim, 7, ln.d_front, Na, ln.pend_k7, ln.pend_dp[0], ln.pend_dp[1], ln.pend_dp[2], ln.pend_dp[3], ln.pend_dp[4], 0, &t);
    ev_end(c, e);
    ln.pend_finish = ln.pend_log = false;
}

static void flush_pending(fl_ctx *c)
{
    Lane &ln = L(c);
    if (ln.pend_yuv) {
        launch_yuv_to_rgb(ln.stream, ln.pend_dim, ln.d_back, ln.d_front);
        std::swap(ln.d_front, ln.d_back);
        ln.pend_yuv = false;
    }
    if (ln.pend_finish) run_de_finish(c, nullptr);
}

int fl_filter(fl_ctx *c, int id, uint32_t w, uint32_t h, const float *p, uint32_t np)
{
    REQUIRE(c, "null ctx");
    HIPCHK(hipSetDevice(c->device));
    fl_dim d; fl_calc_dim(w, h, &d);
    int rc = ensure_fb(c, d);
    if (rc) return rc;
    hipStream_t st = L(c).stream;
    float k7[7];
    EvPair *e = ev_begin(c, c->filt_ev);
    switch (id) {
    case FL_FILT_YUV:
        flush_pending(c);
        L(c).pend_yuv = true; L(c).pend_dim = d;
        break;
    case FL_FILT_BILATERAL: {
        REQUIRE(np >= 5, "bilateral needs sstd,cstd,dstd,dpow,gspeed");
        gauss7(1.0f, k7);
        if (L(c).pend_finish) flush_pending(c);
        L(c).pend_in_mode = L(c).pend_yuv ? 2 : 1;
        L(c).pend_yuv = false;
        L(c).pend_finish = true; L(c).pend_log = false; L(c).pend_dim = d;
        for (int i = 0; i < 5; ++i) L(c).pend_dp[i] = p[i];
        for (int i = 0; i < 7; ++i) L(c).pend_k7[i] = k7[i];
    } break;
    case FL_FILT_LOGSCALE:
        REQUIRE(np >= 2, "logscale needs k1,k2");
        if (L(c).pend_finish && !L(c).pend_log && !L(c).pend_yuv) { L(c).pend_log = true; L(c).pend_k1 = p[0]; L(c).pend_k2 = p[1]; break; }
        flush_pending(c);
        launch_logscale(st, d, L(c).d_front, p[0], p[1]);
        break;
    case FL_FILT_COLORCLIP:
        REQUIRE(np >= 5, "colorclip needs vib,highpow,gam,lin,lingam");
        if (L(c).pend_finish && !L(c).pend_yuv) {
            run_de_finish(c, p);
            break;
        }
        flush_pending(c);
        launch_colorclip(st, d, L(c).d_front, p[0], p[1], p[2], p[3], p[4]);
        break;
    case FL_FILT_SMEARCLIP:
        flush_pending(c);
        REQUIRE(np >= 4, "smearclip needs width,gam_m_1,lin,lingam");
        gauss7(p[0], k7);
        launch_gamma_full_hi(st, d, L(c).d_side, L(c).d_front);
        launch_full_blur(st, d, L(c).d_back, L(c).d_side, 2, 0, k7);
        launch_full_blur(st, d, L(c).d_side, L(c).d_back, 3, 0, k7);
        launch_full_blur(st, d, L(c).d_back, L(c).d_side, 0, 0, k7);
        launch_full_blur(st, d, L(c).d_side, L(c).d_back, 1, 0, k7);
        launch_smearclip(st, d, L(c).d_front, L(c).d_side, p[1], p[2], p[3]);
        break;
    case FL_FILT_HALOCLIP:
        flush_pending(c);
        REQUIRE(np >= 1, "haloclip needs gam_m_1");
        gauss7(1.0f, k7);
        launch_apply_gamma(st, d, L(c).d_blur, L(c).d_front, 0.1f);
        launch_den_blur_1c(st, d, (float *)L(c).d_side, L(c).d_blur, 2, 0, k7);
        launch_den_blur_1c(st, d, L(c).d_blur, (const float *)L(c).d_side, 3, 0, k7);
        launch_haloclip(st, d, L(c).d_front, L(c).d_blur, p[0]);
        break;
    case FL_FILT_PLAINCLIP:
        flush_pending(c);
        REQUIRE(np >= 4, "plainclip needs gam_m_1,lin,lingam,brightness");
        launch_plainclip(st, d, L(c).d_front, p[0], p[1], p[2], p[3]);
        break;
    case FL_FILT_LOGENCODE:
        flush_pending(c);
        REQUIRE(np >= 1, "logencode needs degamma");
        launch_logencode(st, d, L(c).d_back, L(c).d_front, p[0]);
        std::swap(L(c).d_front, L(c).d_back);
        break;
    case FL_FILT_DE: {
        flush_pending(c);
        REQUIRE(np >= 3, "de needs R,Rmin,curve");
        REQUIRE(!(p[0] > (float)FL_DE_MAX_RADIUS), "de: R above 96 px");
        REQUIRE(p[2] > 0.0f, "de: curve must be > 0");
        if (!(p[0] > 0.0f)) break;
        launch_de_adaptive(st, d, L(c).d_front, L(c).d_back, L(c).d_blur, L(c).d_de_tmax, L(c).d_de_sinv,
                           p[0], std::min(std::max(p[1], 0.0f), p[0]), p[2]);
    } break;
    default:
        return fail(FL_E_UNSUPPORTED, "unknown filter id", __FILE__, __LINE__);
    }
    ev_end(c, e);
    HIPCHK(hipGetLastError());
    return FL_OK;
}

size_t fl_output_bytes(uint32_t w, uint32_t h, int fmt)
{
    const size_t n = (size_t)w * h;
    switch (fmt) {
    case FL_OUT_RGBA8: return 4 * n;
    case FL_OUT_RGBA16: return 8 * n;
    case FL_OUT_YUV444P: return 3 * n;
    case FL_OUT_YUV444P10: case FL_OUT_YUV444P12: return 6 * n;
    case FL_OUT_YUV420P10: return 3 * n;
    default: return 0;
    }
}

int fl_output(fl_ctx *c, uint32_t w, uint32_t h, int fmt, void *host_out, uint64_t dev_out)
{
    REQUIRE(c && fl_output_bytes(w, h, fmt) != 0, "bad argument");
    REQUIRE(fmt != FL_OUT_YUV420P10 || (w % 2 == 0 && h % 2 == 0), "4:2:0 needs even width and height");
    HIPCHK(hipSetDevice(c->device));
    fl_dim d; fl_calc_dim(w, h, &d);
    int rc = ensure_fb(c, d);
    if (rc) return rc;
    flush_pending(c);
    void *dst = dev_out ? (void *)(uintptr_t)dev_out : L(c).d_outpix;
    { int rc2 = wait_other(c, 2); if (rc2) return rc2; }
    fl_mwc *rng_out = c->d_rng + (size_t)c->nslots * c->nw * 64 + FL_PAL_H * 256;
    launch_f32_to_rgba(L(c).stream, d, L(c).d_front, rng_out, FL_NOUT, fmt, dst);
    HIPCHK(hipGetLastError());
    HIPCHK(hipEventRecord(L(c).ev_out_done, L(c).stream));
    L(c).out_rec = true;
    if (host_out) HIPCHK(hipMemcpyAsync(host_out, dst, fl_output_bytes(w, h, fmt), hipMemcpyDeviceToHost, L(c).stream));
    if (c->frame_seq) HIPCHK(hipEventRecord(c->ev_end_[(c->frame_seq - 1) % fl_ctx::kFrames], L(c).stream));
    return FL_OK;
}

int fl_sort_u32(fl_ctx *c, uint64_t dst_dev, uint64_t src_dev, uint32_t n, uint32_t lo_bit, uint32_t nbits, int ignore_max,
                uint32_t *nvalid)
{
    REQUIRE(c && dst_dev && src_dev && dst_dev != src_dev, "null or aliased key arrays");
    REQUIRE(nbits >= 1 && nbits <= 10 && lo_bit + nbits <= 32, "a pass sorts 1..10 bits inside the 32-bit key");
    HIPCHK(hipSetDevice(c->device));
    if (n == 0) { if (nvalid) *nvalid = 0; return FL_OK; }
    size_t chunk_words = 0;
    const size_t hist_words = sort_scratch_words(n, nbits, &chunk_words), need = hist_words + chunk_words;
    hipStream_t sst = c->lanes[0].stream;
    if (need > c->sort_words) {
        sync_all(c);
        hipFree(c->d_sort); c->d_sort = nullptr; c->sort_words = 0;
        HIPCHK(hipMalloc(&c->d_sort, need * 4));
        c->sort_words = need;
    }
    uint32_t *chunk_tot = c->d_sort + hist_words, *total_dev = chunk_tot + (chunk_words - 1);
    launch_sort_pass(sst, (uint32_t *)(uintptr_t)dst_dev, (const uint32_t *)(uintptr_t)src_dev, n, lo_bit, nbits,
                     ignore_max, c->d_sort, chunk_tot, total_dev);
    HIPCHK(hipGetLastError());
    if (nvalid) {
        HIPCHK(hipMemcpyAsync(nvalid, total_dev, 4, hipMemcpyDeviceToHost, sst));
        HIPCHK(hipStreamSynchronize(sst));
    }
    return FL_OK;
}

int fl_frame_ms(fl_ctx *c, uint32_t frame_id, float *ms)
{
    REQUIRE(c && ms, "null argument");
    REQUIRE(frame_id < c->frame_seq && c->frame_seq - frame_id <= fl_ctx::kFrames, "frame id no longer tracked");
    const uint32_t k = frame_id % fl_ctx::kFrames;
    HIPCHK(hipEventSynchronize(c->ev_end_[k]));
    HIPCHK(hipEventElapsedTime(ms, c->ev_begin_[k], c->ev_end_[k]));
    return FL_OK;
}

int fl_frame_query(fl_ctx *c, uint32_t frame_id)
{
    REQUIRE(c, "null ctx");
    REQUIRE(frame_id < c->frame_seq && c->frame_seq - frame_id <= fl_ctx::kFrames, "frame id no longer tracked");
    hipError_t e = hipEventQuery(c->ev_end_[frame_id % fl_ctx::kFrames]);
    if (e == hipSuccess) return 1;
    if (e == hipErrorNotReady) { (void)hipGetLastError(); return 0; }
    return fail(FL_E_HIP, "hipEventQuery", __FILE__, __LINE__, e);
}

void *fl_host_alloc(size_t nbytes)
{
    void *p = nullptr;
    if (hipHostMalloc(&p, nbytes, hipHostMallocDefault) != hipSuccess) { (void)hipGetLastError(); return nullptr; }
    return p;
}

void fl_host_free(void *p) { if (p) hipHostFree(p); }

static float sum_ms(std::vector<EvPair> &v)
{
    float t = 0.0f;
    for (auto &p : v) { float ms = 0.0f; if (hipEventElapsedTime(&ms, p.a, p.b) == hipSuccess) t += ms; }
    return t;
}

int fl_timings_reset(fl_ctx *c)
{
    REQUIRE(c, "null ctx");
    sync_all(c);
    c->iter_ev.clear(); c->accum_ev.clear(); c->flush_ev.clear(); c->filt_ev.clear(); c->de_ev.clear(); c->pool_used = 0;
    c->n_spec_launch = c->n_interp_launch = 0;
    return FL_OK;
}

int fl_timings_detail(fl_ctx *c, float ms[6])
{
    REQUIRE(c && ms, "null argument");
    sync_all(c);
    ms[0] = sum_ms(c->iter_ev); ms[1] = sum_ms(c->accum_ev); ms[2] = sum_ms(c->flush_ev);
    ms[3] = sum_ms(c->filt_ev); ms[4] = sum_ms(c->de_ev); ms[5] = 0.0f;
    return FL_OK;
}

int fl_launch_stats(fl_ctx *c, uint32_t out[4])
{
    REQUIRE(c && out, "null argument");
    out[0] = c->n_spec_launch; out[1] = c->n_interp_launch; out[2] = c->nslots; out[3] = (uint32_t)c->nw;
    return FL_OK;
}

int fl_measure_copy(int device, size_t nbytes, int iters, float *ms)
{
    REQUIRE(ms && iters > 0 && nbytes >= 16, "bad argument");
    HIPCHK(hipSetDevice(device));
    if (launch_measure_copy(nbytes, iters, ms)) return fail(FL_E_HIP, "copy measurement (allocation of 2 x nbytes, or the launch)", __FILE__, __LINE__);
    return FL_OK;
}

int fl_timings(fl_ctx *c, float *iter_ms, float *flush_ms, float *filter_ms, uint32_t *nlaunch)
{
    REQUIRE(c, "null ctx");
    sync_all(c);
    if (iter_ms) *iter_ms = sum_ms(c->iter_ev);
    if (flush_ms) *flush_ms = sum_ms(c->accum_ev) + sum_ms(c->flush_ev);
    if (filter_ms) *filter_ms = sum_ms(c->filt_ev);
    if (nlaunch) *nlaunch = (uint32_t)c->iter_ev.size();
    return FL_OK;
}

static int buf_ptr(fl_ctx *c, fl_genome *g, int which, void **p, size_t *cap)
{
    switch (which) {
    case FL_BUF_FRONT: *p = L(c).d_front; *cap = 16 * L(c).nbins; break;
    case FL_BUF_BACK: *p = L(c).d_back; *cap = 16 * L(c).nbins; break;
    case FL_BUF_SIDE: *p = L(c).d_side; *cap = 16 * L(c).nbins; break;
    case FL_BUF_PARAMS: *p = L(c).d_params; *cap = 4 * L(c).params_floats; break;
    case FL_BUF_PALETTE: *p = L(c).d_palette; *cap = 8 * FL_PAL_H * FL_PAL_W; break;
    case FL_BUF_POINTS: *p = c->d_points; *cap = 16 * (size_t)c->nslots * c->nw * 64; break;
    case FL_BUF_SEEDS: *p = c->d_rng; *cap = sizeof(fl_mwc) * (size_t)c->nwalkers; break;
    case FL_BUF_ATOM: *p = L(c).d_atom; *cap = 8 * L(c).nbins; break;
    case FL_BUF_HOT: *p = L(c).d_hot; *cap = 4 * (L(c).nbins / 16); break;
    default: return fail(FL_E_INVAL, "unknown buffer", __FILE__, __LINE__);
    }
    if (!*p) return fail(FL_E_INVAL, "buffer not allocated yet", __FILE__, __LINE__);
    return FL_OK;
}

int fl_read_buffer(fl_ctx *c, fl_genome *g, int which, void *dst, size_t nbytes)
{
    REQUIRE(c && dst, "null argument");
    HIPCHK(hipSetDevice(c->device));
    flush_pending(c);
    void *p; size_t cap;
    int rc = buf_ptr(c, g, which, &p, &cap);
    if (rc) return rc;
    REQUIRE(nbytes <= cap, "read larger than buffer");
    sync_all(c);
    HIPCHK(hipMemcpy(dst, p, nbytes, hipMemcpyDeviceToHost));
    return FL_OK;
}

int fl_buffer_ptr(fl_ctx *c, fl_genome *g, int which, void **dev_ptr, size_t *nbytes)
{
    REQUIRE(c && dev_ptr && nbytes, "null argument");
    HIPCHK(hipSetDevice(c->device));
    flush_pending(c);
    int rc = buf_ptr(c, g, which, dev_ptr, nbytes);
    if (rc) return rc;
    sync_all(c);
    return FL_OK;
}

int fl_buffer_ptr_async(fl_ctx *c, fl_genome *g, int which, void **dev_ptr, size_t *nbytes)
{
    REQUIRE(c && dev_ptr && nbytes, "null argument");
    HIPCHK(hipSetDevice(c->device));
    flush_pending(c);
    return buf_ptr(c, g, which, dev_ptr, nbytes);
}

int fl_reserve(fl_ctx *c, uint32_t w, uint32_t h)
{
    REQUIRE(c && w && h, "bad argument");
    HIPCHK(hipSetDevice(c->device));
    fl_dim d; fl_calc_dim(w, h, &d);
    return ensure_fb(c, d);
}

int fl_stream_dependency(fl_ctx *c, void *stream, int ctx_waits)
{
    REQUIRE(c, "null ctx");
    HIPCHK(hipSetDevice(c->device));
    hipStream_t other = (hipStream_t)stream;
    hipEvent_t &ev = c->dep_ev[c->dep_next++ % fl_ctx::kDepEvents];
    if (!ev) HIPCHK(hipEventCreateWithFlags(&ev, hipEventDisableTiming));
    if (ctx_waits) {
        HIPCHK(hipEventRecord(ev, other));
        HIPCHK(hipStreamWaitEvent(L(c).stream, ev, 0));
    } else {
        flush_pending(c);
        HIPCHK(hipEventRecord(ev, L(c).stream));
        HIPCHK(hipStreamWaitEvent(other, ev, 0));
    }
    return FL_OK;
}

int fl_write_buffer(fl_ctx *c, fl_genome *g, int which, const void *src, size_t nbytes)
{
    REQUIRE(c && src, "null argument");
    HIPCHK(hipSetDevice(c->device));
    flush_pending(c);
    void *p; size_t cap;
    int rc = buf_ptr(c, g, which, &p, &cap);
    if (rc) return rc;
    REQUIRE(nbytes <= cap, "write larger than buffer");
    sync_all(c);
    HIPCHK(hipMemcpy(p, src, nbytes, hipMemcpyHostToDevice));
    if (which == FL_BUF_PARAMS) L(c).params_serial = 0;
    return FL_OK;
}

int fl_debug_clear(fl_ctx *c, uint32_t w, uint32_t h, int reset_points)
{
    REQUIRE(c, "null ctx");
    HIPCHK(hipSetDevice(c->device));
    fl_dim d; fl_calc_dim(w, h, &d);
    int rc = ensure_fb(c, d);
    if (rc) return rc;
    flush_pending(c);
    return do_clear(c, d, reset_points != 0);
}

int fl_debug_iter_launch(fl_ctx *c, fl_genome *g, uint32_t w, uint32_t h, uint32_t round0,
                         uint32_t nrounds, uint32_t fuse, int accum_mode)
{
    REQUIRE(c && g && (accum_mode == FL_ACCUM_ATOMIC || accum_mode == FL_ACCUM_BINNED), "bad argument");
    REQUIRE(L(c).params_floats >= (size_t)c->ntemporal() * g->pstride, "fl_interp has not run for this genome");
    HIPCHK(hipSetDevice(c->device));
    fl_dim d; fl_calc_dim(w, h, &d);
    int rc = ensure_fb(c, d);
    if (rc) return rc;
    c->round_counter = round0;
    HIPCHK(hipMemsetAsync(c->d_counters, 0, 32, L(c).stream));
    return do_iter_launch(c, g, d, nrounds, fuse, true, accum_mode);
}

int fl_debug_flush(fl_ctx *c, uint32_t w, uint32_t h)
{
    REQUIRE(c, "null ctx");
    fl_dim d; fl_calc_dim(w, h, &d);
    int rc = ensure_fb(c, d);
    if (rc) return rc;
    flush_pending(c);
    return do_flush(c, d);
}

int fl_debug_clear_hot(fl_ctx *c, uint32_t w, uint32_t h)
{
    REQUIRE(c && L(c).d_hot, "null ctx");
    fl_dim d; fl_calc_dim(w, h, &d);
    HIPCHK(hipMemsetAsync(L(c).d_hot, 0, 4 * ((size_t)d.ah * d.astride / 16), L(c).stream));
    return FL_OK;
}

struct DevBuf {
    void *p = nullptr;
    ~DevBuf() { if (p) hipFree(p); }
    hipError_t alloc(size_t n) { return hipMalloc(&p, n); }
};

int fl_debug_shuffle(fl_ctx *c, uint32_t round, uint32_t *out256)
{
    REQUIRE(c && out256, "null argument");
    HIPCHK(hipSetDevice(c->device));
    DevBuf d; const size_t n = (size_t)c->nw * 64;
    HIPCHK(d.alloc(4 * n));
    launch_shuffle_tap(L(c).stream, c->nw, (uint32_t *)d.p, round);
    HIPCHK(hipStreamSynchronize(L(c).stream));
    HIPCHK(hipMemcpy(out256, d.p, 4 * n, hipMemcpyDeviceToHost));
    return FL_OK;
}

int fl_debug_apply_xf(fl_ctx *c, fl_genome *g, uint32_t ts, int xfi, uint32_t n, float *xyzw, fl_mwc *rng)
{
    REQUIRE(c && g && xyzw && rng && n > 0 && ts < c->ntemporal(), "bad argument");
    REQUIRE(xfi >= 0 && xfi < g->prog[1] + g->prog[2], "xform index out of range");
    REQUIRE(L(c).params_floats >= (size_t)c->ntemporal() * g->pstride, "fl_interp has not run for this genome");
    HIPCHK(hipSetDevice(c->device));
    DevBuf dp, dr;
    HIPCHK(dp.alloc(16 * (size_t)n));
    HIPCHK(dr.alloc(sizeof(fl_mwc) * (size_t)n));
    HIPCHK(hipMemcpy(dp.p, xyzw, 16 * (size_t)n, hipMemcpyHostToDevice));
    HIPCHK(hipMemcpy(dr.p, rng, sizeof(fl_mwc) * (size_t)n, hipMemcpyHostToDevice));
    launch_apply_xf_tap(L(c).stream, g->d_prog, L(c).d_params, ts, xfi, n, (float4 *)dp.p, (fl_mwc *)dr.p);
    HIPCHK(hipStreamSynchronize(L(c).stream));
    HIPCHK(hipMemcpy(xyzw, dp.p, 16 * (size_t)n, hipMemcpyDeviceToHost));
    HIPCHK(hipMemcpy(rng, dr.p, sizeof(fl_mwc) * (size_t)n, hipMemcpyDeviceToHost));
    return FL_OK;
}

int fl_rtc_compile_check(const int32_t *prog, uint32_t nprog, const int32_t *ops, uint32_t nops, int nw, int count, int acc,
                         char *log, size_t log_bytes)
{
    REQUIRE(prog && ops && nprog >= FL_PROG_HDR && (nw == 4 || nw == 8 || nw == 16) && acc >= 0 && acc <= 3, "bad argument");
    int rc = check_prog(prog, nprog);
    if (rc) return rc;
    const int xo = prog[5], xs = prog[6], vs = prog[7], nrec = prog[1] + prog[2];
    IterSpec spec;
    spec.nxf = prog[1]; spec.has_final = prog[2]; spec.pstride = prog[3]; spec.cdf_off = prog[4];
    spec.xf_off = xo; spec.xf_stride = xs; spec.var_stride = vs;
    spec.nvar.assign(nrec, 0); spec.post.assign(nrec, 0); spec.opac.assign(nrec, 0); spec.vids.assign(nrec, std::vector<int>(16, 0));
    for (uint32_t i = 0; i < nops; ++i) {
        const int32_t *o = ops + 4 * i;
        if (o[0] == FL_OP_OPACITY) {
            const int rel = o[1] - xo;
            REQUIRE(rel >= 0 && rel / xs < prog[1] && rel % xs == 15, "opacity op must write word 15 of a selectable xform record");
        }
        if (o[0] != FL_OP_CONST) continue;
        const int rel = o[1] - xo, rec = rel / xs, w = rel % xs;
        REQUIRE(rel >= 0 && rec < nrec, "structure word outside the xform records");
        if (w == 14) {
            REQUIRE((o[2] >> 10) == 0 && (((o[2] >> 9) & 1) == 0 || rec < prog[1]), "bad structure word");
            spec.nvar[rec] = o[2] & 0xff; spec.post[rec] = (o[2] >> 8) & 1; spec.opac[rec] = (o[2] >> 9) & 1;
        }
        else { const int j = (w - FL_XF_HDR) / vs; if (j >= (int)spec.vids[rec].size()) spec.vids[rec].resize(j + 1, 0); spec.vids[rec][j] = o[2]; }
    }
    std::vector<char> code;
    std::string err;
    rc = rtc_compile(spec, nw, (count & 1) != 0, acc, &code, &err, nullptr, (count & 2) == 0 ? 0u : nw == 8 ? 1u : nw == 16 ? 2u : 0u);
    if (log && log_bytes) { snprintf(log, log_bytes, "%s", rc ? err.c_str() : "ok"); }
    if (rc) return fail(rtc_available() ? FL_E_HIP : FL_E_UNSUPPORTED, "per-genome kernel did not compile", __FILE__, __LINE__);
    return (int)(code.size() > 0 ? FL_OK : FL_E_HIP);
}

int fl_debug_counters(fl_ctx *c, uint64_t out4[4])
{
    REQUIRE(c && out4, "null argument");
    sync_all(c);
    HIPCHK(hipMemcpy(out4, c->d_counters, 32, hipMemcpyDeviceToHost));
    return FL_OK;
}

}
#pragma GCC visibility pop
```

cuburn_amd/csrc/flame_device.h:

```cpp
#pragma once
#ifdef __HIPCC_RTC__
typedef unsigned char uint8_t;
typedef unsigned short uint16_t;
typedef unsigned int uint32_t;
typedef int int32_t;
typedef unsigned long long uint64_t;
typedef long long int64_t;
typedef unsigned long size_t;
#include "flame_hip.h"
#else
#include <hip/hip_runtime.h>
#include <stdint.h>
#include "../../include/flame_hip.h"
#endif

typedef unsigned long long u64;

#define FM_PI 3.14159274101257f
#define FM_PI_2 1.57079637050629f
#define FM_1_PI 0.31830987334251f
#define FM_2_PI 0.63661974668503f
#define FM_LOG2E 1.44269502162933f
#define FM_SQRT2 1.41421353816986f
#define FL_INV255 0.003921568859368562698f

struct mwc_t { uint32_t mul, state, carry; };

__device__ __forceinline__ uint32_t mwc_next(mwc_t &s) {
    u64 t = (u64)s.mul * s.state + s.carry;
    s.state = (uint32_t)t;
    s.carry = (uint32_t)(t >> 32);
    return s.state;
}
__device__ __forceinline__ float mwc_next_01(mwc_t &s) { return (float)mwc_next(s) * (1.0f / 4294967296.0f); }
__device__ __forceinline__ float mwc_next_11(mwc_t &s) { return (float)(int32_t)mwc_next(s) * (1.0f / 2147483648.0f); }

__device__ __forceinline__ void unpack_cell(u64 cell, float &y, float &u, float &v, float &d) {
    uint32_t hi = (uint32_t)(cell >> 32), lo = (uint32_t)cell;
    d = (float)(hi >> 22);
    y = (float)__builtin_amdgcn_ubfe(hi, 4, 18);
    u = (float)(((hi & 0xfu) << 14) | (lo >> 18));
    v = (float)(lo & 0x3ffffu);
}
__device__ __forceinline__ float hot_mult(uint32_t flag) { return flag ? (float)((1u << (flag << 1)) >> 1) : 1.0f; }

__device__ __forceinline__ float frcp(float a) { return __builtin_amdgcn_rcpf(a); }
__device__ __forceinline__ float fdiv(float a, float b) { return a * __builtin_amdgcn_rcpf(b); }
__device__ __forceinline__ float fexp2(float x) { return __builtin_amdgcn_exp2f(x); }
__device__ __forceinline__ float flog2(float x) { return __builtin_amdgcn_logf(x); }
__device__ __forceinline__ float fexp(float x) { return __builtin_amdgcn_exp2f(x * FM_LOG2E); }
__device__ __forceinline__ float flog(float x) { return __builtin_amdgcn_logf(x) * 0.69314718246460f; }
__device__ __forceinline__ float fpow(float x, float y) { return __builtin_amdgcn_exp2f(y * __builtin_amdgcn_logf(x)); }
__device__ __forceinline__ float de_pow(float w, float dpow) { return dpow == 0.0f ? 1.0f : fpow(w, dpow); }
__device__ __forceinline__ float fsqrt(float a) { return __builtin_amdgcn_sqrtf(a); }
__device__ __forceinline__ float fsin(float x) { return __builtin_amdgcn_sinf(__builtin_amdgcn_fractf(x * 0.15915494309189532f)); }
__device__ __forceinline__ float fcos(float x) { return __builtin_amdgcn_cosf(__builtin_amdgcn_fractf(x * 0.15915494309189532f)); }
__device__ __forceinline__ float ftan(float x) { return fsin(x) * frcp(fcos(x)); }

__device__ __forceinline__ uint32_t trunca(float f) {
    float c = fminf(fmaxf(f, -2147483648.0f), 2147483520.0f);
    int32_t i = (int32_t)__builtin_rintf(c);
    if (f >= 2147483648.0f) i = 0x7fffffff;
    return (f != f) ? 0u : (uint32_t)i;
}

#define FL_TILE_W 128u
#define FL_TILE_H_LOG2 6u
#define FL_TILE_H (1u << FL_TILE_H_LOG2)
#define FL_TILE_CELLS (FL_TILE_W * FL_TILE_H)
#define FL_REC_BITS (15u + FL_TILE_H_LOG2)
#ifndef FL_LOG_PACK3
#define FL_LOG_PACK3 1
#endif
__host__ __device__ static inline uint32_t fl_pack3_words(uint32_t batch_records) { return ((batch_records + 2u) / 3u + 1u) & ~1u; }
#define FL_MAX_BINS 2047u
#define FL_TILE_W_WIDE_LOG2 8u
#define FL_MAX_BINS_WIDE 8191u
#define FL_BIN_R_MAX 16

__device__ __forceinline__ uint32_t xcc_id() { return __builtin_amdgcn_s_getreg(((4 - 1) << 11) | 20) & 7; }
```

cuburn_amd/csrc/iter.hip:

```cpp
#include "variations.h"
#ifndef FL_RTC
#include "kernels.h"
#include <hip/hip_ext.h>
#endif

#define FL_CNT_SETS 3
#define FL_CNT_SETS_BIG 2
#define FL_SCATTER_DEPTH 4
#ifndef FL_ITER_MERGE_MAX_XF
#define FL_ITER_MERGE_MAX_XF 4
#endif
#ifndef FL_SORT_FULL_COPY
#define FL_SORT_FULL_COPY 1
#endif
#ifndef FL_SORT_LOCAL_TID
#define FL_SORT_LOCAL_TID 1
#endif

template <int NW>
__device__ __forceinline__ uint32_t shuffle_dest(uint32_t w, uint32_t l, uint32_t phase) {
    uint32_t sh = l + (phase == 1 ? l / NW : 0u) + (phase == 2 ? l / (NW * NW) : 0u);
    return ((w + sh) % NW) * 64u + l;
}

struct XfHead { float f[16]; int vid0; float w0; };
#define FL_XTAB_BYTES 256

__device__ __forceinline__ XfHead load_head(const float *__restrict__ xf) {
    XfHead h;
#pragma unroll
    for (int i = 0; i < 16; ++i) h.f[i] = xf[i];
    h.vid0 = __float_as_int(xf[FL_XF_HDR]);
    h.w0 = xf[FL_XF_HDR + 1];
    return h;
}

__device__ __forceinline__ void opacity_mark(const bool has, const float q, float &c, mwc_t &r)
{
    const uint32_t qb = __float_as_uint(q);
    uint32_t hid = 0u;
    if (has) {
        if (qb - 1u < 0x3f800000u - 1u) hid = mwc_next_01(r) <= q ? 0u : 0x80000000u;
        else if (qb == 0u) hid = 0x80000000u;
    }
    c = __uint_as_float((__float_as_uint(c) & 0x7fffffffu) | hid);
}

__device__ __forceinline__ void apply_xf(const XfHead &h, const float *__restrict__ xf, int var_stride,
                                         float &x, float &y, float &c, mwc_t &r, const bool any_opac = false)
{
    const int word14 = __float_as_int(h.f[14]);
    const int nvar = word14 & 0xff;
    float tx = fmaf(h.f[0], x, fmaf(h.f[1], y, h.f[2]));
    float ty = fmaf(h.f[3], x, fmaf(h.f[4], y, h.f[5]));
    float ox = -0.0f, oy = -0.0f;
    if (nvar > 0) apply_variation(h.vid0, h.w0, xf + FL_XF_HDR + 2, xf, tx, ty, ox, oy, r);
    for (int j = 1; j < nvar; ++j) {
        const float *__restrict__ v = xf + FL_XF_HDR + j * var_stride;
        apply_variation(__float_as_int(v[0]), v[1], v + 2, xf, tx, ty, ox, oy, r);
    }
    if (word14 & 0x100) {
        const float qx = fmaf(h.f[6], ox, fmaf(h.f[7], oy, h.f[8]));
        const float qy = fmaf(h.f[9], ox, fmaf(h.f[10], oy, h.f[11]));
        ox = qx; oy = qy;
    }
    const float csp = h.f[13];
    c = fmaf(c, 1.0f - csp, h.f[12] * csp);
    if (any_opac) opacity_mark((word14 & 0x200) != 0, h.f[15], c, r);
    x = ox; y = oy;
}

#ifdef FL_RTC
#include "flame_spec.h"

constexpr int kTailFirst = FL_XF_HDR + 2, kTailWords = 10;
struct XfTail { float w[kTailWords]; };
struct VTail {
    const float *__restrict__ p; const XfTail *t; int base;
    __device__ __forceinline__ float operator[](int i) const {
        const int wd = base + i;
        return (t && wd >= kTailFirst && wd < kTailFirst + kTailWords) ? t->w[wd - kTailFirst] : p[wd];
    }
};
template <int I, int J>
__device__ __forceinline__ void spec_variations(const float *__restrict__ xf, float w0, float &tx, float &ty,
                                                float &ox, float &oy, mwc_t &r, const XfTail *tl = nullptr)
{
    if constexpr (J < kSpecNvar[I]) {
        constexpr int B = FL_XF_HDR + J * FL_SPEC_VAR_STRIDE;
        const VTail v = {xf, tl, B + 2}, vh = {xf, tl, B};
        apply_variation_body(kSpecVid[I][J], J == 0 ? w0 : vh[1], v, xf, tx, ty, ox, oy, r);
        spec_variations<I, J + 1>(xf, w0, tx, ty, ox, oy, r, tl);
    }
}

__host__ __device__ constexpr bool spec_any_opac() { for (int i = 0; i < FL_SPEC_NXF; ++i) if (kSpecOpac[i] != 0) return true; return false; }
constexpr bool kAnyOpac = spec_any_opac();
template <int I>
__device__ __forceinline__ void spec_opacity(const XfHead &h, float &c, mwc_t &r)
{
    if constexpr (kAnyOpac && I < FL_SPEC_NXF) opacity_mark(kSpecOpac[I] != 0, h.f[15], c, r);
}

template <int I>
__device__ __forceinline__ void spec_apply_xf(const XfHead &h, const float *__restrict__ xf,
                                              float &x, float &y, float &c, mwc_t &r)
{
    float tx = fmaf(h.f[0], x, fmaf(h.f[1], y, h.f[2]));
    float ty = fmaf(h.f[3], x, fmaf(h.f[4], y, h.f[5]));
    float ox = -0.0f, oy = -0.0f;
    spec_variations<I, 0>(xf, h.w0, tx, ty, ox, oy, r);
    if constexpr (kSpecPost[I] != 0) {
        const float qx = fmaf(h.f[6], ox, fmaf(h.f[7], oy, h.f[8]));
        const float qy = fmaf(h.f[9], ox, fmaf(h.f[10], oy, h.f[11]));
        ox = qx; oy = qy;
    }
    const float csp = h.f[13];
    c = fmaf(c, 1.0f - csp, h.f[12] * csp);
    spec_opacity<I>(h, c, r);
    x = ox; y = oy;
}

__host__ __device__ constexpr int spec_resident_sgprs()
{
    int n = 0;
    for (int i = 0; i < FL_SPEC_NXF; ++i) n += 9 + (kSpecPost[i] != 0 ? 6 : 0);
    return n;
}
constexpr bool kSpecResident = FL_SPEC_NXF <= 4 && spec_resident_sgprs() <= 48;
#ifndef FL_HOIST_BUDGET
#define FL_HOIST_BUDGET 12
#endif
__host__ __device__ constexpr int spec_npost() { int n = 0; for (int i = 0; i < FL_SPEC_NXF; ++i) n += kSpecPost[i] != 0 ? 1 : 0; return n; }
constexpr bool kHoistCol = kSpecResident && FL_SPEC_NXF + 2 <= FL_HOIST_BUDGET;
constexpr bool kHoistAff = kHoistCol && 3 * FL_SPEC_NXF + 2 <= FL_HOIST_BUDGET;
constexpr bool kHoistPost = kHoistAff && 3 * FL_SPEC_NXF + 2 + 2 * spec_npost() <= FL_HOIST_BUDGET;
struct XfVec { float xo, yo, cprod, pxo, pyo; };
constexpr bool kTab = !kSpecResident && FL_HOIST_BUDGET >= 12 && FL_SPEC_NXF * 16 <= FL_XTAB_BYTES;
template <int I, class Extra>
__device__ __forceinline__ void spec_apply_xf_tab(const XfHead &h, const float4 &t, const float *__restrict__ xf,
                                                  float &x, float &y, float &c, mwc_t &r, const XfTail *tl, Extra &&extra)
{
    extra();
    float tx = fmaf(h.f[0], x, fmaf(h.f[1], y, t.x));
    float ty = fmaf(h.f[3], x, fmaf(h.f[4], y, t.y));
    float ox = -0.0f, oy = -0.0f;
    spec_variations<I, 0>(xf, h.w0, tx, ty, ox, oy, r, tl);
    if constexpr (kSpecPost[I] != 0) {
        const float qx = fmaf(h.f[6], ox, fmaf(h.f[7], oy, h.f[8]));
        const float qy = fmaf(h.f[9], ox, fmaf(h.f[10], oy, h.f[11]));
        ox = qx; oy = qy;
    }
    c = fmaf(c, t.z, t.w);
    asm volatile("" : "+v"(c));
    spec_opacity<I>(h, c, r);
    x = ox; y = oy;
}
template <int LO, int HI, class Extra>
__device__ __forceinline__ void spec_dispatch_tab(int k, const XfHead &h, const float4 &t, const float *__restrict__ xf,
                                                  float &x, float &y, float &c, mwc_t &r, const XfTail *tl, Extra &&extra)
{
    if constexpr (HI - LO == 1) spec_apply_xf_tab<LO>(h, t, xf, x, y, c, r, tl, extra);
    else {
        constexpr int MID = (LO + HI) / 2;
        if (k < MID) spec_dispatch_tab<LO, MID>(k, h, t, xf, x, y, c, r, tl, extra);
        else spec_dispatch_tab<MID, HI>(k, h, t, xf, x, y, c, r, tl, extra);
    }
}
constexpr bool kHoistFinal = FL_SPEC_FINAL != 0 && FL_HOIST_BUDGET >= 7;
template <int I, bool COL = kHoistCol, bool AFF = kHoistAff, bool POST = kHoistPost>
__device__ __forceinline__ void spec_apply_xf_res(const XfHead &h, const XfVec &v, const float *__restrict__ xf,
                                                  float &x, float &y, float &c, mwc_t &r, const XfTail *tl = nullptr)
{
    float tx = fmaf(h.f[0], x, fmaf(h.f[1], y, AFF ? v.xo : h.f[2]));
    float ty = fmaf(h.f[3], x, fmaf(h.f[4], y, AFF ? v.yo : h.f[5]));
    float ox = -0.0f, oy = -0.0f;
    spec_variations<I, 0>(xf, h.w0, tx, ty, ox, oy, r, tl);
    if constexpr (kSpecPost[I] != 0) {
        const float qx = fmaf(h.f[6], ox, fmaf(h.f[7], oy, POST ? v.pxo : h.f[8]));
        const float qy = fmaf(h.f[9], ox, fmaf(h.f[10], oy, POST ? v.pyo : h.f[11]));
        ox = qx; oy = qy;
    }
    if constexpr (COL) { c = fmaf(c, h.f[13], v.cprod); asm volatile("" : "+v"(c)); }
    else { const float csp = h.f[13]; c = fmaf(c, 1.0f - csp, h.f[12] * csp); }
    spec_opacity<I>(h, c, r);
    x = ox; y = oy;
}
template <int LO, int HI, class Extra>
__device__ __forceinline__ void spec_dispatch_res(int k, const XfHead (&heads)[FL_SPEC_NXF], const XfVec (&hv)[FL_SPEC_NXF], const float *__restrict__ xf0, int xf_stride,
                                                  float &x, float &y, float &c, mwc_t &r, const XfTail (&tails)[FL_SPEC_NXF], Extra &&extra)
{
    if constexpr (HI - LO == 1) { extra(); spec_apply_xf_res<LO>(heads[LO], hv[LO], xf0 + LO * xf_stride, x, y, c, r, &tails[LO]); }
    else {
        constexpr int MID = (LO + HI) / 2;
        if (k < MID) spec_dispatch_res<LO, MID>(k, heads, hv, xf0, xf_stride, x, y, c, r, tails, extra);
        else spec_dispatch_res<MID, HI>(k, heads, hv, xf0, xf_stride, x, y, c, r, tails, extra);
    }
}

template <int LO, int HI, class Extra>
__device__ __forceinline__ void spec_dispatch(int k, const XfHead &h, const float *__restrict__ xf,
                                              float &x, float &y, float &c, mwc_t &r, Extra &&extra)
{
    if constexpr (HI - LO == 1) { extra(); spec_apply_xf<LO>(h, xf, x, y, c, r); }
    else {
        constexpr int MID = (LO + HI) / 2;
        if (k < MID) spec_dispatch<LO, MID>(k, h, xf, x, y, c, r, extra);
        else spec_dispatch<MID, HI>(k, h, xf, x, y, c, r, extra);
    }
}
#endif

__device__ __forceinline__ void drain_if_full(bool ok, u64 old, uint32_t gi, float mult,
                                              u64 *__restrict__ atom, float *__restrict__ out4, uint32_t &n_spill)
{
    if (ok && (uint32_t)(old >> 32) >= (256u << 23)) {
        const u64 cur = __hip_atomic_exchange(atom + gi, 0ull, __ATOMIC_RELAXED, __HIP_MEMORY_SCOPE_AGENT);
        if ((uint32_t)(cur >> 32) != 0u) {
            float yf, uf, vf, df;
            unpack_cell(cur, yf, uf, vf, df);
            const float m255 = mult * FL_INV255;
            float *o = out4 + 4 * (size_t)gi;
            __hip_atomic_fetch_add(o + 0, yf * m255, __ATOMIC_RELAXED, __HIP_MEMORY_SCOPE_AGENT);
            __hip_atomic_fetch_add(o + 1, uf * m255, __ATOMIC_RELAXED, __HIP_MEMORY_SCOPE_AGENT);
            __hip_atomic_fetch_add(o + 2, vf * m255, __ATOMIC_RELAXED, __HIP_MEMORY_SCOPE_AGENT);
            __hip_atomic_fetch_add(o + 3, df * mult, __ATOMIC_RELAXED, __HIP_MEMORY_SCOPE_AGENT);
            ++n_spill;
        }
    }
}

__device__ __forceinline__ void reseed(float &x, float &y, float &c, mwc_t &r) {
    x = mwc_next_11(r); y = mwc_next_11(r); c = mwc_next_01(r);
}

struct BinGeom {
    uint32_t tiles_x;
    uint32_t nbins;
    uint32_t rounds;
    uint32_t nbatch_total;
    uint32_t sub_log2;
};

__device__ __forceinline__ uint32_t wave_incl_scan(uint32_t v, uint32_t) {
    v += (uint32_t)__builtin_amdgcn_update_dpp(0, (int)v, 0x111, 0xf, 0xf, false);
    v += (uint32_t)__builtin_amdgcn_update_dpp(0, (int)v, 0x112, 0xf, 0xf, false);
    v += (uint32_t)__builtin_amdgcn_update_dpp(0, (int)v, 0x114, 0xf, 0xf, false);
    v += (uint32_t)__builtin_amdgcn_update_dpp(0, (int)v, 0x118, 0xf, 0xf, false);
    v += (uint32_t)__builtin_amdgcn_update_dpp(0, (int)v, 0x142, 0xa, 0xf, false);
    v += (uint32_t)__builtin_amdgcn_update_dpp(0, (int)v, 0x143, 0xc, 0xf, false);
    return v;
}

template <int NW, bool COUNT, int ACC, bool SPEC>
__device__ __forceinline__ void
iter_body(unsigned char *smem, const int32_t *__restrict__ prog, const float *__restrict__ params,
          const u64 *__restrict__ palette, fl_mwc *__restrict__ rng, float4 *__restrict__ points,
          const uint32_t *__restrict__ hot, u64 *__restrict__ atom, float *__restrict__ out4,
          u64 *__restrict__ counters, uint32_t astride, uint32_t aheight,
          uint32_t round0, uint32_t nrounds, uint32_t fuse, BinGeom bg,
          uint32_t *__restrict__ bin_log, uint32_t *__restrict__ bin_dir)
{
    constexpr int NT = NW * 64;
    constexpr int SETS = NW == 4 ? FL_CNT_SETS : FL_CNT_SETS_BIG;
    constexpr bool BINNED = ACC == 1 || ACC == 3, WIDE = ACC == 3;
    constexpr bool PACK3 = FL_LOG_PACK3 != 0 && ACC == 1;
    constexpr uint32_t TWL = WIDE ? FL_TILE_W_WIDE_LOG2 : 7u;
    constexpr uint32_t PAY_BITS = TWL + FL_TILE_H_LOG2 + 8u;
    float (*swp)[3][NT] = reinterpret_cast<float (*)[3][NT]>(smem);
    u64 *palrow = reinterpret_cast<u64 *>(smem + 2 * 3 * NT * 4);
    uint32_t *stage = reinterpret_cast<uint32_t *>(smem + 2 * 3 * NT * 4);
    uint16_t *skey = reinterpret_cast<uint16_t *>(stage + bg.rounds * NT);
    uint32_t *cnt = stage + bg.rounds * NT + (WIDE ? bg.rounds * NT / 2 : 0);
    const uint32_t CNTW = (bg.nbins + 1 + 3) & ~3u;
    uint32_t *s_nvalid = cnt + SETS * CNTW;
    uint32_t *tot = s_nvalid + 4;
    float4 *xtab = BINNED ? reinterpret_cast<float4 *>(tot + 128) : reinterpret_cast<float4 *>(palrow + FL_PAL_W);
    uint32_t *my_cnt = cnt + ((threadIdx.x & 63u) % SETS) * CNTW;

    const uint32_t tid = threadIdx.x, w = tid >> 6, l = tid & 63;
#ifdef FL_RTC
    constexpr uint32_t kSubSpec = FL_SPEC_SUB_LOG2;
#else
    constexpr uint32_t kSubSpec = 0;
#endif
    const uint32_t sub_log2 = NW == 4 ? 0u : SPEC ? kSubSpec : bg.sub_log2;
    const bool pair = sub_log2 != 0u;
    const uint32_t half = pair ? (uint32_t)__builtin_amdgcn_readfirstlane((int)(w >> 2)) : 0u;
    const uint32_t slot = blockIdx.x, ts = pair ? (slot << sub_log2) + half : slot, prow = slot * FL_PAL_H / gridDim.x;
#ifdef FL_RTC
    const int nxf = SPEC ? FL_SPEC_NXF : prog[1], has_final = SPEC ? FL_SPEC_FINAL : prog[2], pstride = SPEC ? FL_SPEC_PSTRIDE : prog[3];
    const int cdf_off = SPEC ? FL_SPEC_CDF_OFF : prog[4], xf_off = SPEC ? FL_SPEC_XF_OFF : prog[5];
    const int xf_stride = SPEC ? FL_SPEC_XF_STRIDE : prog[6], var_stride = SPEC ? FL_SPEC_VAR_STRIDE : prog[7];
#else
    const int nxf = prog[1], has_final = prog[2], pstride = prog[3], cdf_off = prog[4];
    const int xf_off = prog[5], xf_stride = prog[6], var_stride = prog[7];
#endif
    const float *__restrict__ P = params + (size_t)ts * pstride;

    if (!BINNED) for (int i = tid; i < FL_PAL_W; i += NT) palrow[i] = palette[prow * FL_PAL_W + i];
    if (BINNED) for (uint32_t i = tid; i < SETS * CNTW; i += NT) cnt[i] = 0;
    uint32_t batch_in_slot = 0;

    const size_t wi = (size_t)slot * NT + tid;
    mwc_t rctx = {rng[wi].mul, rng[wi].state, rng[wi].carry};
    float4 pt = points[wi];
    float x = pt.x, y = pt.y, color = pt.z;

    const float color_dither = 0.49f * mwc_next_11(rctx);
    if (!isfinite(fabsf(x) + fabsf(y))) reseed(x, y, color, rctx);
    __syncthreads();
    const float cam0 = P[0], cam1 = P[1], cam3 = P[3], cam4 = P[4];
    float cam2 = P[2], cam5 = P[5];
#ifdef FL_RTC
    if constexpr (SPEC && FL_HOIST_BUDGET >= 2) asm volatile("" : "+v"(cam2), "+v"(cam5));
#endif
    const float *__restrict__ xf_final = P + xf_off + nxf * xf_stride;
#ifdef FL_RTC
    constexpr bool OPAC = SPEC ? kAnyOpac : true;
#else
    constexpr bool OPAC = true;
#endif
    bool any_opac = false;
    if constexpr (OPAC && SPEC) any_opac = true;
    else if constexpr (OPAC) for (int i = 0; i < nxf; ++i) any_opac |= (__float_as_int(P[xf_off + i * xf_stride + 14]) & 0x200) != 0;
    uint32_t hid_bits = 0u;

    const float cdf_lane = ((int)l < nxf - 1 && l < 63u) ? P[cdf_off + (int)l] : -1.0f;
    auto sel_ok = [&](uint32_t s) -> bool { return (float)s * (1.0f / 4294967296.0f) <= cdf_lane; };
    const bool thr_valid = sel_ok(0u);
    uint32_t thr = 0xffffffffu;
    if (!sel_ok(thr)) {
        uint32_t lo = 0u, hi = 0xffffffffu;
        for (int it = 0; it < 32; ++it) {
            const uint32_t mid = lo + ((hi - lo) >> 1);
            if (sel_ok(mid)) lo = mid; else hi = mid;
        }
        thr = lo;
    }
    auto swap_dest = [&](const uint32_t phase) -> uint32_t {
        return pair ? (w & ~3u) * 64u + shuffle_dest<4>(w & 3u, l, phase) : shuffle_dest<NW>(w, l, phase);
    };
    uint32_t rot0 = swap_dest(round0 % 3u), rot1 = swap_dest((round0 + 1u) % 3u), rot2 = swap_dest((round0 + 2u) % 3u);
    uint32_t n_acc = 0, n_oob = 0, n_drop = 0, n_spill = 0;
    bool pend_ok = false; uint32_t pend_gi = 0; float pend_mult = 1.0f; u64 pend_old = 0;

    const unsigned long long valid_lanes = __ballot(thr_valid);
    auto choose = [&](uint32_t sel) -> int {
        const unsigned long long le = (__ballot(sel <= thr) & valid_lanes) | (1ull << 63);
        return min((int)__builtin_ctzll(le), nxf - 1);
    };
    uint32_t sel_next = __builtin_amdgcn_readfirstlane(mwc_next(rctx));
    int k_next = choose(sel_next);
    const float *__restrict__ xf_next = P + xf_off + k_next * xf_stride;
#ifdef FL_RTC
    constexpr bool RESIDENT = SPEC && kSpecResident;
    XfHead heads[FL_SPEC_NXF];
    XfVec hv[FL_SPEC_NXF] = {};
    XfTail tails[FL_SPEC_NXF] = {};
    if constexpr (RESIDENT) {
#pragma unroll
        for (int i = 0; i < FL_SPEC_NXF; ++i) {
            heads[i] = load_head(P + xf_off + i * xf_stride);
#pragma unroll
            for (int k = 0; k < kTailWords; ++k) tails[i].w[k] = (P + xf_off + i * xf_stride)[kTailFirst + k];
            if constexpr (kHoistCol) {
                const float csp = heads[i].f[13];
                hv[i].cprod = heads[i].f[12] * csp;
                asm volatile("" : "+v"(hv[i].cprod));
                heads[i].f[13] = __int_as_float(__builtin_amdgcn_readfirstlane(__float_as_int(1.0f - csp)));
            }
            if constexpr (kHoistAff) { hv[i].xo = heads[i].f[2]; hv[i].yo = heads[i].f[5]; asm volatile("" : "+v"(hv[i].xo), "+v"(hv[i].yo)); }
            if constexpr (kHoistPost) { hv[i].pxo = heads[i].f[8]; hv[i].pyo = heads[i].f[11]; asm volatile("" : "+v"(hv[i].pxo), "+v"(hv[i].pyo)); }
        }
    }
    XfHead hfin_res = {};
    XfTail tfin = {};
    XfVec vfin = {};
    if constexpr (SPEC && kHoistFinal) {
        hfin_res = load_head(xf_final);
#pragma unroll
        for (int k = 0; k < kTailWords; ++k) tfin.w[k] = xf_final[kTailFirst + k];
        const float csp = hfin_res.f[13];
        vfin.cprod = hfin_res.f[12] * csp;
        vfin.xo = hfin_res.f[2]; vfin.yo = hfin_res.f[5];
        asm volatile("" : "+v"(vfin.cprod), "+v"(vfin.xo), "+v"(vfin.yo));
        hfin_res.f[13] = __int_as_float(__builtin_amdgcn_readfirstlane(__float_as_int(1.0f - csp)));
        if constexpr (kSpecPost[FL_SPEC_NXF] != 0) { vfin.pxo = hfin_res.f[8]; vfin.pyo = hfin_res.f[11]; asm volatile("" : "+v"(vfin.pxo), "+v"(vfin.pyo)); }
    }
#else
    constexpr bool RESIDENT = false;
#endif
    XfHead hnext = RESIDENT ? XfHead{} : load_head(xf_next);
#ifdef FL_RTC
    XfTail tail_next = {};
    if constexpr (SPEC && kTab) {
#pragma unroll
        for (int i = 0; i < kTailWords; ++i) tail_next.w[i] = xf_next[kTailFirst + i];
    }
#endif
    float4 tcur = make_float4(0.0f, 0.0f, 0.0f, 0.0f);
#ifdef FL_RTC
    if constexpr (SPEC && kTab) {
        const uint32_t th = pair ? tid & 255u : tid;
        if ((int)th < FL_SPEC_NXF) {
            const float *__restrict__ rr = P + xf_off + (int)th * xf_stride;
            const float csp = rr[13];
            xtab[half * 16u + th] = make_float4(rr[2], rr[5], 1.0f - csp, rr[12] * csp);
        }
        __syncthreads();
        tcur = xtab[half * 16u + k_next];
    }
#endif

    uint32_t par = 0;
    auto advance = [&](const uint32_t dst, auto &&extra) __attribute__((always_inline)) {
        __builtin_amdgcn_s_setprio(2);
        if (!isfinite(fabsf(x) + fabsf(y))) reseed(x, y, color, rctx);

        const int k_cur = k_next;
        const float *__restrict__ xf_cur = xf_next;
#ifdef FL_RTC
        XfTail tail = tail_next;
#endif
        sel_next = __builtin_amdgcn_readfirstlane(mwc_next(rctx));
        k_next = choose(sel_next);
        xf_next = P + xf_off + k_next * xf_stride;
#ifdef FL_RTC
        if constexpr (RESIDENT) spec_dispatch_res<0, FL_SPEC_NXF>(k_cur, heads, hv, P + xf_off, xf_stride, x, y, color, rctx, tails, extra);
        else if constexpr (SPEC && kTab) spec_dispatch_tab<0, FL_SPEC_NXF>(k_cur, hnext, tcur, xf_cur, x, y, color, rctx, &tail, extra);
        else if constexpr (SPEC) spec_dispatch<0, FL_SPEC_NXF>(k_cur, hnext, xf_cur, x, y, color, rctx, extra);
        else
#endif
        { extra(); apply_xf(hnext, xf_cur, var_stride, x, y, color, rctx, any_opac); }
        if constexpr (!RESIDENT) hnext = load_head(xf_next);
#ifdef FL_RTC
        if constexpr (SPEC && kTab) {
#pragma unroll
            for (int i = 0; i < kTailWords; ++i) tail_next.w[i] = xf_next[kTailFirst + i];
        }
#endif
        (void)k_cur; (void)xf_cur;

        {
            swp[par][0][dst] = x; swp[par][1][dst] = y; swp[par][2][dst] = color;
            __syncthreads();
            x = swp[par][0][tid]; y = swp[par][1][tid]; color = swp[par][2][tid];
            if constexpr (OPAC) if (any_opac) { hid_bits = __float_as_uint(color); color = fabsf(color); }
#ifdef FL_RTC
            if constexpr (SPEC && kTab) tcur = xtab[half * 16u + k_next];
#endif
            __builtin_amdgcn_s_setprio(0);
            par ^= 1u;
        }
    };
    const uint32_t nfuse = min(fuse, nrounds);
#ifdef FL_RTC
    constexpr bool SPLIT_FUSE = !SPEC || FL_SPEC_NXF <= 9;
#else
    constexpr bool SPLIT_FUSE = true;
#endif
    constexpr bool ROT3 = SPLIT_FUSE;
    uint32_t ph = 0;
    auto next_dst = [&]() __attribute__((always_inline)) -> uint32_t {
        const uint32_t dst = rot0;
        rot0 = rot1; rot1 = rot2; rot2 = dst;
        return dst;
    };
    auto rounds = [&](uint32_t from, uint32_t to, auto body) __attribute__((always_inline)) {
        if constexpr (ROT3) {
            uint32_t i = from;
            while (i < to) {
                if (ph == 0u) { body(rot0, i); ph = 1u; if (++i == to) break; }
                if (ph == 1u) { body(rot1, i); ph = 2u; if (++i == to) break; }
                body(rot2, i); ph = 0u; ++i;
            }
        } else {
            for (uint32_t i = from; i < to; ++i) body(next_dst(), i);
        }
    };
#ifdef FL_RTC
    constexpr bool MERGE = BINNED && SPEC && SPLIT_FUSE && FL_SPEC_NXF <= FL_ITER_MERGE_MAX_XF;
#else
    constexpr bool MERGE = false;
#endif
    auto plot_head = [&](float &cx, float &cy, float &cf) __attribute__((always_inline)) {
        float fx = x, fy = y, fc = color;
#ifdef FL_RTC
        if constexpr (SPEC) {
            if constexpr (kHoistFinal) spec_apply_xf_res<FL_SPEC_NXF, true, true, true>(hfin_res, vfin, xf_final, fx, fy, fc, rctx, &tfin);
            else if constexpr (FL_SPEC_FINAL != 0) { const XfHead hfin = load_head(xf_final); spec_apply_xf<FL_SPEC_NXF>(hfin, xf_final, fx, fy, fc, rctx); }
        } else
#endif
        if (has_final) { const XfHead hfin = load_head(xf_final); apply_xf(hfin, xf_final, var_stride, fx, fy, fc, rctx); }
        cx = fmaf(cam0, fx, fmaf(cam1, fy, cam2));
        cy = fmaf(cam3, fx, fmaf(cam4, fy, cam5));
        cf = fminf(fmaxf(fmaf(fc, 255.0f, color_dither), 0.0f), 255.0f) + 8388608.0f;
        if constexpr (OPAC) if (any_opac) cf = __uint_as_float((__float_as_uint(cf) & 0x7fffffffu) | (hid_bits & 0x80000000u));
        if constexpr (MERGE) asm volatile("" : "+v"(cx), "+v"(cy), "+v"(cf));
    };
    auto plot_rest = [&](const float cx, const float cy, const float cf, const uint32_t staged) __attribute__((always_inline)) {
        const uint32_t ix = __float_as_uint(cx + 12582912.0f) - 0x4b400000u;
        const uint32_t iy = __float_as_uint(cy + 12582912.0f) - 0x4b400000u;
        bool ok = (ix < astride) & (iy < aheight);
        if constexpr (OPAC) {
            if (any_opac) {
                const bool hidden = (__float_as_uint(cf) >> 31) != 0u;
                if (COUNT) { n_drop += hidden; n_oob += !hidden & !ok; }
                ok &= !hidden;
            } else if (COUNT) n_oob += !ok;
        } else
        if (COUNT) n_oob += !ok;
        const uint32_t gi = ok ? iy * astride + ix : 0u;

        float mult = 1.0f;
        if (ok && !BINNED) {
            const uint32_t flag = (hot[gi >> 4] >> ((gi & 15u) << 1)) & 3u;
            if (flag) {
                mult = hot_mult(flag);
                if (mwc_next_01(rctx) > frcp(mult)) { ok = false; if (COUNT) ++n_drop; }
            }
        }
        const uint32_t cbits = __float_as_uint(cf);
        const int ci = (int)((cbits - 0x4b000000u) & 0xffu);
        const u64 val = BINNED ? 0ull : palrow[ci];

        if (ACC == 0) {
            drain_if_full(pend_ok, pend_old, pend_gi, pend_mult, atom, out4, n_spill);
            pend_ok = ok; pend_gi = gi; pend_mult = mult;
            if (ok) pend_old = __hip_atomic_fetch_add(atom + gi, val, __ATOMIC_RELAXED, __HIP_MEMORY_SCOPE_AGENT);
        } else if (BINNED) {
            const uint32_t bin = ok ? __umul24(iy >> FL_TILE_H_LOG2, bg.tiles_x) + (ix >> TWL) : bg.nbins;
            const uint32_t t1 = ((iy & (FL_TILE_H - 1u)) << TWL) | (ix & ((1u << TWL) - 1u));
            const uint32_t t2 = WIDE ? t1 : (bin << (TWL + FL_TILE_H_LOG2)) | t1;
            const uint32_t rec = __builtin_amdgcn_perm(t2, cbits, 0x06050400u);
            if (WIDE) skey[staged * NT + tid] = (uint16_t)bin;
            stage[staged * NT + tid] = rec;
            if constexpr (OPAC) { if (!any_opac || ok) __hip_atomic_fetch_add(my_cnt + bin, 1u, __ATOMIC_RELAXED, __HIP_MEMORY_SCOPE_WORKGROUP); }
            else __hip_atomic_fetch_add(my_cnt + bin, 1u, __ATOMIC_RELAXED, __HIP_MEMORY_SCOPE_WORKGROUP);
        } else {
            pend_old += ok ? val + gi : 0ull;
        }
        if (COUNT) n_acc += ok;
    };
    auto no_extra = []() __attribute__((always_inline)) {};
    if (SPLIT_FUSE) rounds(0u, MERGE && nfuse < nrounds ? nfuse + 1u : nfuse, [&](uint32_t dst, uint32_t) __attribute__((always_inline)) { advance(dst, no_extra); });
    uint32_t fuse_left = SPLIT_FUSE ? 0u : nfuse;
    for (uint32_t rd = SPLIT_FUSE ? nfuse : 0u; rd < nrounds;) {
    const uint32_t blen = fuse_left ? fuse_left : BINNED ? min(bg.rounds, nrounds - rd) : nrounds - rd;
    const bool plotting = fuse_left == 0u;
    fuse_left = 0u;
    if constexpr (MERGE) {
        const uint32_t last = rd + blen >= nrounds ? 1u : 0u;
        rounds(0u, blen - last, [&](const uint32_t dst, const uint32_t staged) __attribute__((always_inline)) {
            float fx, fy, fc;
            plot_head(fx, fy, fc);
            advance(dst, [&]() __attribute__((always_inline)) { plot_rest(fx, fy, fc, staged); });
        });
        if (last) { float fx, fy, fc; plot_head(fx, fy, fc); plot_rest(fx, fy, fc, blen - 1u); }
    } else
    rounds(0u, blen, [&](const uint32_t dst, const uint32_t staged) __attribute__((always_inline)) {
        advance(dst, no_extra);
        if (!SPLIT_FUSE && !plotting) return;
        float fx, fy, fc;
        plot_head(fx, fy, fc);
        plot_rest(fx, fy, fc, staged);
    });
    rd += blen;
    if (BINNED && plotting) {
            auto sort_batch = [&](const uint32_t staged) __attribute__((always_inline)) {
#if FL_SORT_LOCAL_TID
                uint32_t tid_local = threadIdx.x;
                asm volatile("" : "+v"(tid_local));
                const uint32_t tid = tid_local, l = tid & 63u;
                const uint32_t w = (uint32_t)__builtin_amdgcn_readfirstlane((int)(tid >> 6));
#endif
                const uint32_t batch_id = slot * (bg.nbatch_total / gridDim.x) + batch_in_slot;
                __syncthreads();
                uint32_t r2[FL_BIN_R_MAX], k2[FL_BIN_R_MAX];
                auto has_record = [&](const uint32_t k) __attribute__((always_inline)) -> bool {
                    if constexpr (OPAC) { if (any_opac && k == bg.nbins) return false; }
                    return k != 0xffffffffu;
                };
#pragma unroll
                for (int q = 0; q < FL_BIN_R_MAX; ++q) {
                    const bool have = (uint32_t)q < staged;
                    r2[q] = have ? stage[q * NT + tid] : 0u;
                    k2[q] = !have ? 0xffffffffu : WIDE ? (uint32_t)skey[q * NT + tid] : r2[q] >> PAY_BITS;
                }
                const uint32_t nchunk = (bg.nbins + 64u) >> 6;
                if (nchunk <= 8u) {
                    if (w == 0) {
                        uint32_t running = 0;
                        for (uint32_t c0 = 0; c0 <= bg.nbins; c0 += 64) {
                            const uint32_t b = c0 + l;
                            uint32_t vs[SETS], v = 0;
#pragma unroll
                            for (int t = 0; t < SETS; ++t) { vs[t] = b <= bg.nbins ? cnt[t * CNTW + b] : 0u; v += vs[t]; }
                            const uint32_t incl = wave_incl_scan(v, l);
                            const uint32_t excl = incl - v + running;
                            if (b <= bg.nbins) {
                                uint32_t at = excl;
#pragma unroll
                                for (int t = 0; t < SETS; ++t) { cnt[t * CNTW + b] = at; at += vs[t]; }
                            }
                            if (b < bg.nbins) bin_dir[(size_t)b * bg.nbatch_total + batch_id] = (excl << 16) | v;
                            if (b == bg.nbins) *s_nvalid = excl;
                            running += (uint32_t)__builtin_amdgcn_readlane((int)incl, 63);
                        }
                    }
                } else {
                for (uint32_t c = w; c < nchunk; c += NW) {
                    const uint32_t b = c * 64u + l;
                    uint32_t v = 0;
#pragma unroll
                    for (int t = 0; t < SETS; ++t) v += b <= bg.nbins ? cnt[t * CNTW + b] : 0u;
                    const uint32_t incl = wave_incl_scan(v, l);
                    if (l == 63u) tot[c] = incl;
                }
                __syncthreads();
                {
                    const uint32_t t0 = l < nchunk ? tot[l] : 0u, t1 = 64u + l < nchunk ? tot[64u + l] : 0u;
                    const uint32_t i0 = wave_incl_scan(t0, l);
                    const uint32_t i1 = wave_incl_scan(t1, l) + (uint32_t)__builtin_amdgcn_readlane((int)i0, 63);
                    for (uint32_t cv = w; cv < nchunk; cv += NW) {
                        const uint32_t c = (uint32_t)__builtin_amdgcn_readfirstlane((int)cv);
                        const uint32_t base = c < 64u ? (uint32_t)__builtin_amdgcn_readlane((int)(i0 - t0), c)
                                                      : (uint32_t)__builtin_amdgcn_readlane((int)(i1 - t1), c - 64u);
                        const uint32_t b = c * 64u + l;
                        uint32_t vs[SETS], v = 0;
#pragma unroll
                        for (int t = 0; t < SETS; ++t) { vs[t] = b <= bg.nbins ? cnt[t * CNTW + b] : 0u; v += vs[t]; }
                        const uint32_t excl = wave_incl_scan(v, l) - v + base;
                        if (b <= bg.nbins) {
                            uint32_t at = excl;
#pragma unroll
                            for (int t = 0; t < SETS; ++t) { cnt[t * CNTW + b] = at; at += vs[t]; }
                            if (b < bg.nbins) bin_dir[(size_t)b * bg.nbatch_total + batch_id] = (excl << 16) | v;
                            else *s_nvalid = excl;
                        }
                    }
                }
                }
                __syncthreads();
#pragma unroll
                for (int q0 = 0; q0 < FL_BIN_R_MAX; q0 += FL_SCATTER_DEPTH) {
                    if ((uint32_t)q0 >= staged) break;
                    uint32_t pos[FL_SCATTER_DEPTH];
#pragma unroll
                    for (int q = 0; q < FL_SCATTER_DEPTH; ++q)
                        if (has_record(k2[q0 + q]))
                            pos[q] = __hip_atomic_fetch_add(my_cnt + k2[q0 + q], 1u, __ATOMIC_RELAXED, __HIP_MEMORY_SCOPE_WORKGROUP);
#pragma unroll
                    for (int q = 0; q < FL_SCATTER_DEPTH; ++q)
                        if (has_record(k2[q0 + q])) stage[pos[q]] = r2[q0 + q] & ((1u << PAY_BITS) - 1u);
                }
                __syncthreads();
                const uint32_t nvalid = *s_nvalid;
                if constexpr (PACK3) {
                    typedef uint32_t u32x2_ __attribute__((ext_vector_type(2)));
                    u32x2_ *d2 = reinterpret_cast<u32x2_ *>(bin_log) + (size_t)batch_id * fl_pack3_words(bg.rounds * NT);
                    const uint32_t nwords = (nvalid + 2u) / 3u;
                    for (uint32_t i = tid; i < nwords; i += NT) {
                        const uint32_t a = stage[3u * i], b = stage[3u * i + 1u], c3 = stage[3u * i + 2u];
                        u32x2_ o;
                        o.x = a | (b << 21); o.y = (b >> 11) | (c3 << 10);
                        __builtin_nontemporal_store(o, d2 + i);
                    }
                } else {
                uint4 *dst = reinterpret_cast<uint4 *>(bin_log + (size_t)batch_id * bg.rounds * NT);
                {
                    typedef uint32_t u32x4_ __attribute__((ext_vector_type(4)));
                    const u32x4_ *s4 = reinterpret_cast<const u32x4_ *>(stage);
                    u32x4_ *d4 = reinterpret_cast<u32x4_ *>(dst);
                    for (uint32_t i = tid; i * 4 < nvalid; i += NT) __builtin_nontemporal_store(s4[i], d4 + i);
                }
                }
                for (uint32_t i = tid; i < SETS * CNTW; i += NT) cnt[i] = 0;
                ++batch_in_slot;
                __syncthreads();
            };
#if FL_SORT_FULL_COPY
            if (blen == (uint32_t)FL_BIN_R_MAX) sort_batch((uint32_t)FL_BIN_R_MAX); else
#endif
            sort_batch(blen);
    }
    }

    if (ACC == 0) drain_if_full(pend_ok, pend_old, pend_gi, pend_mult, atom, out4, n_spill);
    else if (pend_old == 0x123456789abcdefull) atom[0] = pend_old;
    {
        uint32_t tid_end = threadIdx.x;
        asm volatile("" : "+v"(tid_end));
        const size_t wj = (size_t)slot * NT + tid_end;
        points[wj] = make_float4(x, y, color, 0.0f);
        rng[wj].mul = rctx.mul; rng[wj].state = rctx.state; rng[wj].carry = rctx.carry;
    }

    if (COUNT) {
        atomicAdd(counters + 0, (u64)n_acc);
        atomicAdd(counters + 1, (u64)n_oob);
        atomicAdd(counters + 2, (u64)n_drop);
        atomicAdd(counters + 3, (u64)n_spill);
    }
}

#define FL_ITER_ARGS const int32_t *__restrict__ prog, const float *__restrict__ params, \
       const u64 *__restrict__ palette, fl_mwc *__restrict__ rng, float4 *__restrict__ points, \
       const uint32_t *__restrict__ hot, u64 *__restrict__ atom, float *__restrict__ out4, \
       u64 *__restrict__ counters, uint32_t astride, uint32_t aheight, \
       uint32_t round0, uint32_t nrounds, uint32_t fuse, BinGeom bg, \
       uint32_t *__restrict__ bin_log, uint32_t *__restrict__ bin_dir
#define FL_ITER_PASS prog, params, palette, rng, points, hot, atom, out4, counters, astride, aheight, round0, nrounds, fuse, bg, bin_log, bin_dir

#ifdef FL_RTC
extern "C" __global__ void __launch_bounds__(FL_SPEC_NW * 64) k_iter_spec(FL_ITER_ARGS)
{
    extern __shared__ __attribute__((aligned(16))) unsigned char smem[];
    iter_body<FL_SPEC_NW, FL_SPEC_COUNT != 0, FL_SPEC_ACC, true>(smem, FL_ITER_PASS);
}
#else
template <int NW, bool COUNT, int ACC>
__global__ void __launch_bounds__(NW * 64, NW == 4 ? 6 : NW == 8 ? 3 : 1) k_iter(FL_ITER_ARGS)
{
    extern __shared__ __attribute__((aligned(16))) unsigned char smem[];
    iter_body<NW, COUNT, ACC, false>(smem, FL_ITER_PASS);
}

__global__ void __launch_bounds__(256)
k_apply_xf_tap(const int32_t *__restrict__ prog, const float *__restrict__ params, uint32_t ts, int xfi,
               uint32_t n, float4 *__restrict__ pts, fl_mwc *__restrict__ rng)
{
    const uint32_t i = blockIdx.x * 256u + threadIdx.x;
    if (i >= n) return;
    const float *__restrict__ P = params + (size_t)ts * prog[3];
    mwc_t r = {rng[i].mul, rng[i].state, rng[i].carry};
    float4 p = pts[i];
    const float *__restrict__ xf = P + prog[5] + xfi * prog[6];
    const XfHead h = load_head(xf);
    apply_xf(h, xf, prog[7], p.x, p.y, p.z, r);
    pts[i] = p;
    rng[i].mul = r.mul; rng[i].state = r.state; rng[i].carry = r.carry;
}

void launch_apply_xf_tap(hipStream_t st, const int32_t *prog, const float *params, uint32_t ts, int xfi,
                         uint32_t n, float4 *pts, fl_mwc *rng)
{
    hipLaunchKernelGGL(k_apply_xf_tap, dim3((n + 255) / 256), dim3(256), 0, st, prog, params, ts, xfi, n, pts, rng);
}

template <int NW>
__global__ void __launch_bounds__(NW * 64) k_shuffle_tap(uint32_t *out, uint32_t round)
{
    __shared__ uint32_t s[NW * 64];
    const uint32_t tid = threadIdx.x;
    s[shuffle_dest<NW>(tid >> 6, tid & 63, round % 3u)] = tid;
    __syncthreads();
    out[tid] = s[tid];
}

__global__ void __launch_bounds__(256)
k_flush(u64 *__restrict__ atom, float4 *__restrict__ out, uint32_t *__restrict__ hot, uint32_t nbins, int use_hot)
{
    const uint32_t gi = blockIdx.x * 256u + threadIdx.x;
    if (gi >= nbins) return;
    const uint32_t sh = (gi & 15u) << 1;
    const uint32_t flag = use_hot ? (hot[gi >> 4] >> sh) & 3u : 0u;
    const float mult = hot_mult(flag);
    const u64 cell = __builtin_nontemporal_load(atom + gi);
    __builtin_nontemporal_store(0ull, atom + gi);
    float yf, uf, vf, df;
    unpack_cell(cell, yf, uf, vf, df);
    float4 o = out[gi];
    const float m255 = mult * FL_INV255;
    o.w = fmaf(df, mult, o.w);
    o.x = fmaf(yf, m255, o.x);
    o.y = fmaf(uf, m255, o.y);
    o.z = fmaf(vf, m255, o.z);
    out[gi] = o;
    uint32_t nf = (uint32_t)(o.w > 128.0f) + (uint32_t)(o.w > 512.0f) + (uint32_t)(o.w > 2048.0f);
    uint32_t word = nf << sh;
    word |= __shfl_xor(word, 1);
    word |= __shfl_xor(word, 2);
    word |= __shfl_xor(word, 4);
    word |= __shfl_xor(word, 8);
    if ((gi & 15u) == 0) hot[gi >> 4] = word;
}

static size_t iter_lds_bytes(int nw, int acc, uint32_t rounds, uint32_t nbins, uint32_t sub_log2)
{
    size_t nt = (size_t)nw * 64, b = 2 * 3 * nt * 4;
    if (acc == 1 || acc == 3) b += (size_t)rounds * nt * (acc == 3 ? 6 : 4) + (nw == 4 ? FL_CNT_SETS : FL_CNT_SETS_BIG) * (size_t)((nbins + 1 + 3) & ~3u) * 4 + 16
             + 128 * 4;
    else b += FL_PAL_W * 8;
    return b + ((size_t)FL_XTAB_BYTES << sub_log2);
}

void launch_iter(hipStream_t st, int nw, bool count, int acc, uint32_t nslots,
                 const int32_t *prog, const float *params, const u64 *palette, fl_mwc *rng,
                 float4 *points, const uint32_t *hot, u64 *atom, float *out4, u64 *counters,
                 uint32_t astride, uint32_t aheight, uint32_t round0, uint32_t nrounds, uint32_t fuse,
                 uint32_t tiles_x, uint32_t nbins, uint32_t rounds_per_batch, uint32_t nbatch_total,
                 uint32_t *log, uint32_t *dir, hipEvent_t ev_start, hipEvent_t ev_stop, uint32_t sub_log2)
{
    if (sub_log2 != 0u && (4 << sub_log2) != nw) abort();
    BinGeom bg = {tiles_x, nbins, rounds_per_batch, nbatch_total, sub_log2};
    const size_t lds = iter_lds_bytes(nw, acc, rounds_per_batch, nbins, sub_log2);
#define LAUNCH(NW, C, A) do { \
        static unsigned long long attr_done = 0; \
        ensure_max_dynamic_lds((const void *)k_iter<NW, C, A>, attr_done); \
         \
        hipExtLaunchKernelGGL((k_iter<NW, C, A>), dim3(nslots), dim3(NW * 64), lds, st, ev_start, ev_stop, 0, prog, params, palette, \
        rng, points, hot, atom, out4, counters, astride, aheight, round0, nrounds, fuse, bg, log, dir); } while (0)
#define LAUNCH_NW(C, A) do { if (nw == 4) LAUNCH(4, C, A); else if (nw == 8) LAUNCH(8, C, A); else LAUNCH(16, C, A); } while (0)
    if (acc == 2) LAUNCH_NW(false, 2);
    else if (acc == 1) { if (count) LAUNCH_NW(true, 1); else LAUNCH_NW(false, 1); }
    else if (acc == 3) { if (count) LAUNCH_NW(true, 3); else LAUNCH_NW(false, 3); }
    else { if (count) LAUNCH_NW(true, 0); else LAUNCH_NW(false, 0); }
#undef LAUNCH_NW
#undef LAUNCH
}

void launch_iter_fn(hipStream_t st, hipFunction_t fn, int nw, int acc, uint32_t nslots,
                    const int32_t *prog, const float *params, const u64 *palette, fl_mwc *rng,
                    float4 *points, const uint32_t *hot, u64 *atom, float *out4, u64 *counters,
                    uint32_t astride, uint32_t aheight, uint32_t round0, uint32_t nrounds, uint32_t fuse,
                    uint32_t tiles_x, uint32_t nbins, uint32_t rounds_per_batch, uint32_t nbatch_total,
                    uint32_t *log, uint32_t *dir, hipEvent_t ev_start, hipEvent_t ev_stop, uint32_t sub_log2)
{
    if (sub_log2 != 0u && (4 << sub_log2) != nw) abort();
    BinGeom bg = {tiles_x, nbins, rounds_per_batch, nbatch_total, sub_log2};
    const size_t lds = iter_lds_bytes(nw, acc, rounds_per_batch, nbins, sub_log2);
    void *args[] = {&prog, &params, &palette, &rng, &points, &hot, &atom, &out4, &counters, &astride, &aheight,
                    &round0, &nrounds, &fuse, &bg, &log, &dir};
    (void)hipExtModuleLaunchKernel(fn, nslots * (uint32_t)nw * 64, 1, 1, (uint32_t)nw * 64, 1, 1, lds, st, args, nullptr, ev_start, ev_stop, 0);
}

void launch_flush(hipStream_t st, u64 *atom, float4 *out, uint32_t *hot, uint32_t nbins, bool use_hot)
{
    hipLaunchKernelGGL(k_flush, dim3((nbins + 255) / 256), dim3(256), 0, st, atom, out, hot, nbins, use_hot ? 1 : 0);
}

__global__ void __launch_bounds__(256)
k_clear_frame(float4 *__restrict__ front, u64 *__restrict__ atom, uint32_t *__restrict__ hot, u64 *__restrict__ counters,
              float4 *__restrict__ points, uint32_t nbins, uint32_t npoints)
{
    const uint32_t i = blockIdx.x * 256u + threadIdx.x;
    if (i < nbins) {
        front[i] = make_float4(0.0f, 0.0f, 0.0f, 0.0f);
        atom[i] = 0ull;
        if ((i & 15u) == 0u) hot[i >> 4] = 0u;
    }
    if (i < npoints) {
        const float nanf_ = __uint_as_float(0x7fc00000u);
        points[i] = make_float4(nanf_, nanf_, nanf_, nanf_);
    }
    if (i < 4u) counters[i] = 0ull;
}

void launch_clear_frame(hipStream_t st, float4 *front, u64 *atom, uint32_t *hot, u64 *counters, float4 *points,
                        uint32_t nbins, uint32_t npoints)
{
    const uint32_t n = nbins > npoints ? nbins : npoints;
    hipLaunchKernelGGL(k_clear_frame, dim3((n + 255) / 256), dim3(256), 0, st, front, atom, hot, counters, points, nbins, npoints);
}

void launch_shuffle_tap(hipStream_t st, int nw, uint32_t *out, uint32_t round)
{
    if (nw == 4) hipLaunchKernelGGL(k_shuffle_tap<4>, dim3(1), dim3(256), 0, st, out, round);
    else if (nw == 8) hipLaunchKernelGGL(k_shuffle_tap<8>, dim3(1), dim3(512), 0, st, out, round);
    else hipLaunchKernelGGL(k_shuffle_tap<16>, dim3(1), dim3(1024), 0, st, out, round);
}
#endif
```

cuburn_amd/csrc/kernels.h:

```cpp
#pragma once
#include <hip/hip_runtime.h>
#include <stdint.h>
#include "../../include/flame_hip.h"

typedef unsigned long long u64;

static inline void ensure_max_dynamic_lds(const void *fn, unsigned long long &done)
{
    int dev = 0;
    if (hipGetDevice(&dev) != hipSuccess || dev < 0 || dev > 63) dev = 63;
    if (done >> dev & 1ull) return;
    hipFuncSetAttribute(fn, hipFuncAttributeMaxDynamicSharedMemorySize, 160 * 1024);
    if (dev != 63) done |= 1ull << dev;
}

void launch_iter(hipStream_t st, int nw, bool count, int acc, uint32_t nslots,
                 const int32_t *prog, const float *params, const u64 *palette, fl_mwc *rng,
                 float4 *points, const uint32_t *hot, u64 *atom, float *out4, u64 *counters,
                 uint32_t astride, uint32_t aheight, uint32_t round0, uint32_t nrounds, uint32_t fuse,
                 uint32_t tiles_x, uint32_t nbins, uint32_t rounds_per_batch, uint32_t nbatch_total,
                 uint32_t *log, uint32_t *dir,
                 hipEvent_t ev_start = nullptr, hipEvent_t ev_stop = nullptr, uint32_t sub_log2 = 0);
void launch_flush(hipStream_t st, u64 *atom, float4 *out, uint32_t *hot, uint32_t nbins, bool use_hot);
void launch_clear_frame(hipStream_t st, float4 *front, u64 *atom, uint32_t *hot, u64 *counters, float4 *points,
                        uint32_t nbins, uint32_t npoints);
void launch_shuffle_tap(hipStream_t st, int nw, uint32_t *out, uint32_t round);
void launch_apply_xf_tap(hipStream_t st, const int32_t *prog, const float *params, uint32_t ts, int xfi,
                         uint32_t n, float4 *pts, fl_mwc *rng);

#include <string>
#include <vector>
struct IterSpec {
    int nxf = 0, has_final = 0, pstride = 0, cdf_off = 0, xf_off = 0, xf_stride = 0, var_stride = 0;
    std::vector<int> nvar, post, opac;
    std::vector<std::vector<int>> vids;
};
bool rtc_available();
unsigned rtc_epoch();
int rtc_compile(const IterSpec &spec, int nw, bool count, int acc, std::vector<char> *code, std::string *err, const char *extra_opt = nullptr, uint32_t sub_log2 = 0);
int rtc_iter_kernel(int device, const IterSpec &spec, int nw, uint32_t nslots, bool count, int acc, hipFunction_t *fn, std::string *err, uint32_t sub_log2 = 0);
void launch_iter_fn(hipStream_t st, hipFunction_t fn, int nw, int acc, uint32_t nslots,
                    const int32_t *prog, const float *params, const u64 *palette, fl_mwc *rng,
                    float4 *points, const uint32_t *hot, u64 *atom, float *out4, u64 *counters,
                    uint32_t astride, uint32_t aheight, uint32_t round0, uint32_t nrounds, uint32_t fuse,
                    uint32_t tiles_x, uint32_t nbins, uint32_t rounds_per_batch, uint32_t nbatch_total,
                    uint32_t *log, uint32_t *dir, hipEvent_t ev_start, hipEvent_t ev_stop, uint32_t sub_log2 = 0);

void launch_accum_tiles(hipStream_t st, const uint32_t *log, const uint32_t *dir, const u64 *palette,
                        u64 *atom, float *out4, uint32_t tiles_x, uint32_t nbins, uint32_t nparts,
                        uint32_t nbatch_total, uint32_t batch_records, uint32_t nslots,
                        uint32_t astride, uint32_t aheight, bool wide);

void launch_interp_palette(hipStream_t st, fl_mwc *rng_pal, const float *ptimes, const float4 *pals,
                           float ts, float tstep, u64 *out);
void launch_interp_params(hipStream_t st, float *params, const float *times, const float *knots,
                          const int32_t *ops, uint32_t nops, uint32_t pstride, uint32_t nts, float ts, float tstep,
                          fl_dim dim, bool zero_first);

void launch_yuv_to_rgb(hipStream_t st, fl_dim d, float4 *dst, const float4 *src);
void launch_den_blur_1c(hipStream_t st, fl_dim d, float *dst, const float *src, int pattern, int upsample, const float *coefs7);
void launch_full_blur(hipStream_t st, fl_dim d, float4 *dst, const float4 *src, int pattern, int upsample, const float *coefs7);
void launch_logscale(hipStream_t st, fl_dim d, float4 *buf, float k1, float k2);
void launch_colorclip(hipStream_t st, fl_dim d, float4 *buf, float vib, float highpow, float gam, float lin, float lingam);
void launch_gamma_full_hi(hipStream_t st, fl_dim d, float4 *dst, const float4 *src);
void launch_smearclip(hipStream_t st, fl_dim d, float4 *buf, const float4 *smear, float gam_m_1, float lin, float lingam);
void launch_apply_gamma(hipStream_t st, fl_dim d, float *dst, const float4 *src, float gamma);
void launch_haloclip(hipStream_t st, fl_dim d, float4 *buf, const float *den, float gam_m_1);
void launch_plainclip(hipStream_t st, fl_dim d, float4 *buf, float gam_m_1, float lin, float lingam, float brightness);
void launch_logencode(hipStream_t st, fl_dim d, float4 *dst, const float4 *src, float degamma);

struct DeTail { int do_log; float k1, k2; int do_clip; float vib, highpow, gam, lin, lingam; int order; };
void launch_de_dir(hipStream_t st, fl_dim d, int pattern, float4 *Nout, const float4 *N, const float *coefs7,
                   float sstd, float cstd, float dstd, float dpow, float gspeed, int in_mode = 1, const DeTail *tail = nullptr);

void launch_de_adaptive(hipStream_t st, fl_dim d, float4 *buf, float4 *stage_c, float *stage_a, uint32_t *tmax,
                        const float *sinv, float R, float Rmin, float curve);
size_t de_adaptive_tiles(fl_dim d);
void de_adaptive_norms(float *out);

void launch_f32_to_rgba(hipStream_t st, fl_dim d, const float4 *src, fl_mwc *rng, uint32_t nrng, int fmt, void *dst);

int launch_measure_copy(size_t nbytes, int iters, float *ms);

int launch_sort_pass(hipStream_t st, uint32_t *dst, const uint32_t *src, uint32_t n, uint32_t lo_bit, uint32_t nbits,
                     int ignore_max, uint32_t *hist, uint32_t *chunk_tot, uint32_t *total_dev);
size_t sort_scratch_words(uint32_t n, uint32_t nbits, size_t *chunk_words);
```

Measured before the change: 208,100 Msamples/s.

## Fuse final binned-accumulator flush into first bilateral DE pass

For binned accumulation, the last flush of the packed atom cells into the float histogram is deferred. The first directional DE pass (pattern 0) now reads the atom cells directly and adds them to each pixel on load, which removes a separate full-frame read-modify-write pass. The atom buffer is then marked dirty and cleared lazily, either at the next frame's clear or when it is exposed through the API. The clear kernel is also split into private and shared parts so the private clear can be issued before waiting on the other lane. The cost is extra per-tap load and unpack work in the DE gather, a smaller B2 grouping to limit register pressure, and more complex pending-state bookkeeping.

```diff
diff --git a/cuburn_amd/csrc/de.hip b/cuburn_amd/csrc/de.hip
--- a/cuburn_amd/csrc/de.hip
+++ b/cuburn_amd/csrc/de.hip
@@ -11,7 +11,22 @@
     float4 *p;
     __device__ __forceinline__ float4 ld(uint32_t i) const { return const_cast<const float4 *>(p)[i]; }
     __device__ __forceinline__ void st(uint32_t i, float4 v) const { p[i] = v; }
+    static constexpr int B2_GROUP = 7;
 };
+struct DeImgCells {
+    const float4 *p;
+    const u64 *cells;
+    __device__ __forceinline__ float4 ld(uint32_t i) const { return flush_px(p[i], cells[i], hot_mult(0u)); }
+    static constexpr int B2_GROUP = 3;
+};
+template <int IN, class F>
+__device__ __forceinline__ void de_with_img(const float4 *p, const u64 *cells, F &&f)
+{
+    if constexpr (IN != 0) {
+        if (cells) { f(DeImgCells{p, cells}); return; }
+    }
+    f(DeImgPlain{const_cast<float4 *>(p)});
+}
 struct DeCoefs { float k[7]; float k2[19]; };
 struct DeSpatial { float s[16]; };
 
@@ -128,12 +143,32 @@
 __device__ float de_b12_global(const IMG &N, const fl_dim &d, int cx, int cy, const DeCoefs &k, float &b1)
 {
     float den = 0.0f;
+    if constexpr (IMG::B2_GROUP >= 7) {
 #pragma unroll
     for (int i = 0; i < 7; ++i) {
         const int x = de_clampi(cx + de_dx(P, 2 * (i - 3)), 0, (int)d.astride - 1), y = de_clampi(cy + de_dy(P, 2 * (i - 3)), 0, (int)d.ah - 1);
         const float v = de_b1_global<P>(N, d, x, y, k);
         if (i == 3) b1 = v;
         den += v * k.k[i];
+    }
+    } else {
+    constexpr int GRP = IMG::B2_GROUP;
+#pragma unroll 1
+    for (int i0 = 0; i0 < 7; i0 += GRP) {
+        float v[GRP];
+#pragma unroll
+        for (int g = 0; g < GRP; ++g) {
+            const int i = min(i0 + g, 6);
+            const int x = de_clampi(cx + de_dx(P, 2 * (i - 3)), 0, (int)d.astride - 1), y = de_clampi(cy + de_dy(P, 2 * (i - 3)), 0, (int)d.ah - 1);
+            v[g] = de_b1_global<P>(N, d, x, y, k);
+        }
+#pragma unroll
+        for (int g = 0; g < GRP; ++g) {
+            if (i0 + g >= 7) break;
+            if (i0 + g == 3) b1 = v[g];
+            den += v[g] * k.k[i0 + g];
+        }
+    }
     }
     return den;
 }
@@ -314,7 +349,8 @@
 template <int P, int IN, int OUT>
 __global__ void __launch_bounds__(DeGeo<P>::NT, DeGeo<P>::MINW)
 k_de_dir(fl_dim d, float4 *__restrict__ Nout_, const float4 *__restrict__ N_, DeCoefs kc, DeSpatial spk,
-         float cs2, float ads, float dpow, float gspeed, uint32_t tiles_y, uint32_t ntiles, uint32_t tiles_x, uint32_t magic, DeTail tail)
+         float cs2, float ads, float dpow, float gspeed, uint32_t tiles_y, uint32_t ntiles, uint32_t tiles_x, uint32_t magic, DeTail tail,
+         const u64 *__restrict__ cells)
 {
     using G = DeGeo<P>;
     static_assert(2 * G::NPX * 4 <= G::NPXB * 16, "the preparation planes must fit into plane B's space");
@@ -325,7 +361,7 @@
     float *s1 = sW + G::NPX;
     float *sF1 = s1 + G::NPX, *sF2 = sF1 + G::NF;
     float *sWf = reinterpret_cast<float *>(smem + (size_t)(G::NPXA + G::NPXB) * 16);
-    const DeImgPlain N = {const_cast<float4 *>(N_)}, Nout = {Nout_};
+    const DeImgPlain Nout = {Nout_};
 
     const uint32_t per_xcd = (ntiles + 7u) / 8u, xcd = blockIdx.x & 7u;
     int tx, ty;
@@ -386,6 +422,7 @@
     if (G::HOIST && !border) {
         float4 tq[G::NIT];
         DE_S_THREAD();
+        de_with_img<IN>(N_, cells, [&](const auto &N) __attribute__((always_inline)) {
 #pragma unroll
         for (int it = 0; it < G::NIT; ++it) {
             int ul, vl;
@@ -393,6 +430,7 @@
             const int gx = bx0 + (((ul - G::HU) * G::K) >> 1) + vl - G::HV, gy = by0 + ul - G::HU;
             tq[it] = DE_IN_PX(N.ld((uint32_t)(gy * (int)d.astride + gx)));
         }
+        });
 #pragma unroll
         for (int it = 0; it < G::NIT; ++it) {
             int idx, ul, vl;
@@ -424,6 +462,7 @@
     float4 tn[G::NIT];
     {
     DE_S_THREAD();
+    de_with_img<IN>(N_, cells, [&](const auto &N) __attribute__((always_inline)) {
     if (G::ROWWISE && !border) {
         const int u0 = sr0 - G::HU;
         const uint32_t g0 = (uint32_t)((by0 + u0) * (int)d.astride + bx0 + ((u0 * G::K) >> 1) + sc0 - G::HV);
@@ -444,7 +483,8 @@
         tn[it] = DE_IN_PX(N.ld((uint32_t)(gy * (int)d.astride + gx)));
     }
     }
-    if (border) {
+    });
+    if (border) de_with_img<IN>(N_, cells, [&](const auto &N) __attribute__((always_inline)) {
         const int x0a = bx0 - G::HV, nrows_top = min(G::ROWS, G::HU - by0), first_bot = max(0, ymax + 1 - (by0 - G::HU));
         int tlo = 1, thi = 0, blo = 1, bhi = 0;
         if (nrows_top > 0) {
@@ -473,7 +513,7 @@
                 sF1[e] = b1;
             }
         }
-    }
+    });
 #pragma unroll
     for (int it = 0; it < G::NIT; ++it) {
         int idx, ul, vl;
@@ -598,7 +638,7 @@
 
 template <int P, int IN, int OUT>
 static void launch_de_dir_one(hipStream_t st, fl_dim d, float4 *Nout, const float4 *N, DeCoefs kc, DeSpatial spk,
-                              float cs2, float ads, float dpow, float gspeed, DeTail tail)
+                              float cs2, float ads, float dpow, float gspeed, DeTail tail, const u64 *cells)
 {
     using G = DeGeo<P>;
     static_assert(G::LDS * (G::MINW * 256 / G::NT) <= 160 * 1024, "LDS must allow MINW waves per SIMD");
@@ -610,11 +650,11 @@
     const uint32_t divisor = tail.order == 0 ? tiles_y : tiles_x, magic = (uint32_t)(0x100000000ull / divisor) + 1u;
     if ((unsigned long long)(ntiles + gran) * divisor >= 0x100000000ull) abort();
     hipLaunchKernelGGL((k_de_dir<P, IN, OUT>), dim3(gran * ((ntiles + gran - 1) / gran)), dim3(G::NT), G::LDS, st, d, Nout, N, kc, spk,
-                       cs2, ads, dpow, gspeed, tiles_y, ntiles, tiles_x, magic, tail);
+                       cs2, ads, dpow, gspeed, tiles_y, ntiles, tiles_x, magic, tail, cells);
 }
 
 void launch_de_dir(hipStream_t st, fl_dim d, int pattern, float4 *Nout, const float4 *N, const float *coefs7,
-                   float sstd, float cstd, float dstd, float dpow, float gspeed, int in_mode, const DeTail *tail)
+                   float sstd, float cstd, float dstd, float dpow, float gspeed, int in_mode, const DeTail *tail, const u64 *cells)
 {
     DeCoefs kc;
     for (int i = 0; i < 7; ++i) kc.k[i] = coefs7[i];
@@ -636,7 +676,7 @@
     none.order = order;
     DeTail tl = tail ? *tail : none;
     tl.order = order;
-#define DE(P, I, O) launch_de_dir_one<P, I, O>(st, d, Nout, N, kc, spk, cs2, ads, dpow, gspeed, tl)
+#define DE(P, I, O) launch_de_dir_one<P, I, O>(st, d, Nout, N, kc, spk, cs2, ads, dpow, gspeed, tl, (P) == 0 ? cells : nullptr)
     switch (pattern) {
     case 0:
         if (in_mode == 2) DE(0, 2, 0); else if (in_mode == 1) DE(0, 1, 0); else abort();
diff --git a/cuburn_amd/csrc/flame_abi.hip b/cuburn_amd/csrc/flame_abi.hip
--- a/cuburn_amd/csrc/flame_abi.hip
+++ b/cuburn_amd/csrc/flame_abi.hip
@@ -49,6 +49,8 @@
     hipEvent_t ev_out_done = nullptr;
     bool interp_rec = false, iter_rec = false, out_rec = false;
     bool pend_yuv = false, pend_finish = false, pend_log = false;
+    bool pend_flush = false, pend_cells = false, atom_dirty = false;
+    fl_dim pend_flush_dim = {0, 0, 0, 0, 0};
     float pend_k1 = 0.0f, pend_k2 = 0.0f;
     int pend_in_mode = 0;
     float pend_dp[5] = {0, 0, 0, 0, 0}, pend_k7[7] = {0, 0, 0, 0, 0, 0, 0};
@@ -180,13 +182,16 @@
     L(c).d_hot = nullptr; L(c).d_outpix = nullptr; L(c).d_de_tmax = nullptr; L(c).d_de_sinv = nullptr;
     L(c).nbins = 0; L(c).outpix_bytes = 0;
     L(c).pend_yuv = L(c).pend_finish = L(c).pend_log = false;
+    L(c).pend_flush = L(c).pend_cells = L(c).atom_dirty = false;
 }
 
 static int ensure_fb(fl_ctx *c, const fl_dim &d)
 {
     size_t nbins = (size_t)d.ah * d.astride, ob = (size_t)d.w * d.h * 8;
     if (L(c).nbins >= nbins && L(c).outpix_bytes >= ob) return FL_OK;
+    if (L(c).nbins) flush_pending(c);
     hipStreamSynchronize(L(c).stream);
+    if (L(c).aux) hipStreamSynchronize(L(c).aux);
     free_fb(c);
     hipError_t e;
     if ((e = hipMalloc(&L(c).d_front, 16 * nbins)) || (e = hipMalloc(&L(c).d_back, 16 * nbins)) ||
@@ -528,11 +533,17 @@
     return FL_OK;
 }
 
-static int do_clear(fl_ctx *c, const fl_dim &d, bool reset_points)
+static int do_clear_private(fl_ctx *c, const fl_dim &d)
 {
     size_t nbins = (size_t)d.ah * d.astride;
-    launch_clear_frame(L(c).stream, L(c).d_front, L(c).d_atom, L(c).d_hot, c->d_counters, c->d_points, (uint32_t)nbins,
-                       reset_points ? c->nslots * (uint32_t)c->nw * 64u : 0u);
+    launch_clear_frame(L(c).stream, L(c).d_front, L(c).d_atom, L(c).d_hot, (uint32_t)nbins);
+    L(c).atom_dirty = false;
+    HIPCHK(hipGetLastError());
+    return FL_OK;
+}
+static int do_clear_shared(fl_ctx *c, bool reset_points)
+{
+    launch_clear_shared(L(c).stream, c->d_counters, c->d_points, reset_points ? c->nslots * (uint32_t)c->nw * 64u : 0u);
     HIPCHK(hipGetLastError());
     return FL_OK;
 }
@@ -646,9 +657,11 @@
     fl_dim d; fl_calc_dim(w, h, &d);
     int rc = ensure_fb(c, d);
     if (rc) return rc;
+    L(c).pend_flush = false;
     flush_pending(c);
+    if ((rc = do_clear_private(c, d))) return rc;
     if ((rc = wait_other(c, 1))) return rc;
-    if ((rc = do_clear(c, d, true))) return rc;
+    if ((rc = do_clear_shared(c, true))) return rc;
     const uint32_t nt = (uint32_t)c->nw * 64;
     const double per_round = (double)c->nslots * nt;
     uint64_t rounds = (uint64_t)ceil(nsamples / per_round);
@@ -687,7 +700,8 @@
         const int buf = pipelined ? (int)(k & 1u) : 0;
         if (pipelined && k >= 2) HIPCHK(hipStreamWaitEvent(L(c).stream, L(c).ev_ac[buf], 0));
         if ((rc = do_iter_launch(c, g, d, (uint32_t)n + f, f, false, accum_mode, buf, drain))) return rc;
-        if ((rc = do_flush(c, d, accum_mode != FL_ACCUM_BINNED, drain))) return rc;
+        if (accum_mode == FL_ACCUM_BINNED && rounds == n) { L(c).pend_flush = true; L(c).pend_flush_dim = d; }
+        else if ((rc = do_flush(c, d, accum_mode != FL_ACCUM_BINNED, drain))) return rc;
         if (pipelined) HIPCHK(hipEventRecord(L(c).ev_ac[buf], drain));
         rounds -= n;
         batch += batch / 2;
@@ -716,7 +730,9 @@
                 clip ? clip[2] : 0.f, clip ? clip[3] : 0.f, clip ? clip[4] : 0.f};
     EvPair *e = ev_begin(c, c->de_ev);
     float4 *Na = ln.d_back, *Nb = ln.d_front;
-    launch_de_dir(ln.stream, ln.pend_dim, 0, Na, Nb, ln.pend_k7, ln.pend_dp[0], ln.pend_dp[1], ln.pend_dp[2], ln.pend_dp[3], ln.pend_dp[4], ln.pend_in_mode, nullptr);
+    launch_de_dir(ln.stream, ln.pend_dim, 0, Na, Nb, ln.pend_k7, ln.pend_dp[0], ln.pend_dp[1], ln.pend_dp[2], ln.pend_dp[3], ln.pend_dp[4], ln.pend_in_mode, nullptr,
+                  ln.pend_cells ? ln.d_atom : nullptr);
+    if (ln.pend_cells) { ln.pend_cells = false; ln.atom_dirty = true; }
     for (int pat = 1; pat < 7; ++pat) {
         launch_de_dir(ln.stream, ln.pend_dim, pat, Nb, Na, ln.pend_k7, ln.pend_dp[0], ln.pend_dp[1], ln.pend_dp[2], ln.pend_dp[3], ln.pend_dp[4]);
         std::swap(Na, Nb);
@@ -729,12 +745,26 @@
 static void flush_pending(fl_ctx *c)
 {
     Lane &ln = L(c);
+    if (ln.pend_flush) {
+        ln.pend_flush = false;
+        do_flush(c, ln.pend_flush_dim, false);
+    }
     if (ln.pend_yuv) {
         launch_yuv_to_rgb(ln.stream, ln.pend_dim, ln.d_back, ln.d_front);
         std::swap(ln.d_front, ln.d_back);
         ln.pend_yuv = false;
     }
     if (ln.pend_finish) run_de_finish(c, nullptr);
+}
+
+static int settle_atom(fl_ctx *c)
+{
+    flush_pending(c);
+    if (L(c).atom_dirty) {
+        HIPCHK(hipMemsetAsync(L(c).d_atom, 0, 8 * L(c).nbins, L(c).stream));
+        L(c).atom_dirty = false;
+    }
+    return FL_OK;
 }
 
 int fl_filter(fl_ctx *c, int id, uint32_t w, uint32_t h, const float *p, uint32_t np)
@@ -749,13 +779,18 @@
     EvPair *e = ev_begin(c, c->filt_ev);
     switch (id) {
     case FL_FILT_YUV:
-        flush_pending(c);
+        if (L(c).pend_yuv || L(c).pend_finish) flush_pending(c);
         L(c).pend_yuv = true; L(c).pend_dim = d;
         break;
     case FL_FILT_BILATERAL: {
         REQUIRE(np >= 5, "bilateral needs sstd,cstd,dstd,dpow,gspeed");
         gauss7(1.0f, k7);
         if (L(c).pend_finish) flush_pending(c);
+        if (L(c).pend_flush) {
+            const fl_dim &fd = L(c).pend_flush_dim, &yd = L(c).pend_dim;
+            if (fd.astride == d.astride && fd.ah == d.ah && (!L(c).pend_yuv || (yd.astride == d.astride && yd.ah == d.ah))) { L(c).pend_flush = false; L(c).pend_cells = true; }
+            else flush_pending(c);
+        }
         L(c).pend_in_mode = L(c).pend_yuv ? 2 : 1;
         L(c).pend_yuv = false;
         L(c).pend_finish = true; L(c).pend_log = false; L(c).pend_dim = d;
@@ -976,7 +1011,7 @@
     case FL_BUF_PALETTE: *p = L(c).d_palette; *cap = 8 * FL_PAL_H * FL_PAL_W; break;
     case FL_BUF_POINTS: *p = c->d_points; *cap = 16 * (size_t)c->nslots * c->nw * 64; break;
     case FL_BUF_SEEDS: *p = c->d_rng; *cap = sizeof(fl_mwc) * (size_t)c->nwalkers; break;
-    case FL_BUF_ATOM: *p = L(c).d_atom; *cap = 8 * L(c).nbins; break;
+    case FL_BUF_ATOM: { int rc = settle_atom(c); if (rc) return rc; } *p = L(c).d_atom; *cap = 8 * L(c).nbins; break;
     case FL_BUF_HOT: *p = L(c).d_hot; *cap = 4 * (L(c).nbins / 16); break;
     default: return fail(FL_E_INVAL, "unknown buffer", __FILE__, __LINE__);
     }
@@ -1066,7 +1101,8 @@
     int rc = ensure_fb(c, d);
     if (rc) return rc;
     flush_pending(c);
-    return do_clear(c, d, reset_points != 0);
+    if ((rc = do_clear_private(c, d))) return rc;
+    return do_clear_shared(c, reset_points != 0);
 }
 
 int fl_debug_iter_launch(fl_ctx *c, fl_genome *g, uint32_t w, uint32_t h, uint32_t round0,
@@ -1078,6 +1114,7 @@
     fl_dim d; fl_calc_dim(w, h, &d);
     int rc = ensure_fb(c, d);
     if (rc) return rc;
+    if ((rc = settle_atom(c))) return rc;
     c->round_counter = round0;
     HIPCHK(hipMemsetAsync(c->d_counters, 0, 32, L(c).stream));
     return do_iter_launch(c, g, d, nrounds, fuse, true, accum_mode);
@@ -1089,7 +1126,7 @@
     fl_dim d; fl_calc_dim(w, h, &d);
     int rc = ensure_fb(c, d);
     if (rc) return rc;
-    flush_pending(c);
+    if ((rc = settle_atom(c))) return rc;
     return do_flush(c, d);
 }
 
diff --git a/cuburn_amd/csrc/flame_device.h b/cuburn_amd/csrc/flame_device.h
--- a/cuburn_amd/csrc/flame_device.h
+++ b/cuburn_amd/csrc/flame_device.h
@@ -44,6 +44,17 @@
 }
 __device__ __forceinline__ float hot_mult(uint32_t flag) { return flag ? (float)((1u << (flag << 1)) >> 1) : 1.0f; }
 
+__device__ __forceinline__ float4 flush_px(float4 o, u64 cell, float mult) {
+    float yf, uf, vf, df;
+    unpack_cell(cell, yf, uf, vf, df);
+    const float m255 = mult * FL_INV255;
+    o.w = fmaf(df, mult, o.w);
+    o.x = fmaf(yf, m255, o.x);
+    o.y = fmaf(uf, m255, o.y);
+    o.z = fmaf(vf, m255, o.z);
+    return o;
+}
+
 __device__ __forceinline__ float frcp(float a) { return __builtin_amdgcn_rcpf(a); }
 __device__ __forceinline__ float fdiv(float a, float b) { return a * __builtin_amdgcn_rcpf(b); }
 __device__ __forceinline__ float fexp2(float x) { return __builtin_amdgcn_exp2f(x); }
diff --git a/cuburn_amd/csrc/iter.hip b/cuburn_amd/csrc/iter.hip
--- a/cuburn_amd/csrc/iter.hip
+++ b/cuburn_amd/csrc/iter.hip
@@ -769,14 +769,7 @@
     const float mult = hot_mult(flag);
     const u64 cell = __builtin_nontemporal_load(atom + gi);
     __builtin_nontemporal_store(0ull, atom + gi);
-    float yf, uf, vf, df;
-    unpack_cell(cell, yf, uf, vf, df);
-    float4 o = out[gi];
-    const float m255 = mult * FL_INV255;
-    o.w = fmaf(df, mult, o.w);
-    o.x = fmaf(yf, m255, o.x);
-    o.y = fmaf(uf, m255, o.y);
-    o.z = fmaf(vf, m255, o.z);
+    const float4 o = flush_px(out[gi], cell, mult);
     out[gi] = o;
     uint32_t nf = (uint32_t)(o.w > 128.0f) + (uint32_t)(o.w > 512.0f) + (uint32_t)(o.w > 2048.0f);
     uint32_t word = nf << sh;
@@ -842,8 +835,7 @@
 }
 
 __global__ void __launch_bounds__(256)
-k_clear_frame(float4 *__restrict__ front, u64 *__restrict__ atom, uint32_t *__restrict__ hot, u64 *__restrict__ counters,
-              float4 *__restrict__ points, uint32_t nbins, uint32_t npoints)
+k_clear_frame(float4 *__restrict__ front, u64 *__restrict__ atom, uint32_t *__restrict__ hot, uint32_t nbins)
 {
     const uint32_t i = blockIdx.x * 256u + threadIdx.x;
     if (i < nbins) {
@@ -851,6 +843,12 @@
         atom[i] = 0ull;
         if ((i & 15u) == 0u) hot[i >> 4] = 0u;
     }
+}
+
+__global__ void __launch_bounds__(256)
+k_clear_shared(u64 *__restrict__ counters, float4 *__restrict__ points, uint32_t npoints)
+{
+    const uint32_t i = blockIdx.x * 256u + threadIdx.x;
     if (i < npoints) {
         const float nanf_ = __uint_as_float(0x7fc00000u);
         points[i] = make_float4(nanf_, nanf_, nanf_, nanf_);
@@ -858,11 +856,15 @@
     if (i < 4u) counters[i] = 0ull;
 }
 
-void launch_clear_frame(hipStream_t st, float4 *front, u64 *atom, uint32_t *hot, u64 *counters, float4 *points,
-                        uint32_t nbins, uint32_t npoints)
-{
-    const uint32_t n = nbins > npoints ? nbins : npoints;
-    hipLaunchKernelGGL(k_clear_frame, dim3((n + 255) / 256), dim3(256), 0, st, front, atom, hot, counters, points, nbins, npoints);
+void launch_clear_frame(hipStream_t st, float4 *front, u64 *atom, uint32_t *hot, uint32_t nbins)
+{
+    hipLaunchKernelGGL(k_clear_frame, dim3((nbins + 255) / 256), dim3(256), 0, st, front, atom, hot, nbins);
+}
+
+void launch_clear_shared(hipStream_t st, u64 *counters, float4 *points, uint32_t npoints)
+{
+    const uint32_t n = npoints > 4u ? npoints : 4u;
+    hipLaunchKernelGGL(k_clear_shared, dim3((n + 255) / 256), dim3(256), 0, st, counters, points, npoints);
 }
 
 void launch_shuffle_tap(hipStream_t st, int nw, uint32_t *out, uint32_t round)
diff --git a/cuburn_amd/csrc/kernels.h b/cuburn_amd/csrc/kernels.h
--- a/cuburn_amd/csrc/kernels.h
+++ b/cuburn_amd/csrc/kernels.h
@@ -22,8 +22,8 @@
                  uint32_t *log, uint32_t *dir,
                  hipEvent_t ev_start = nullptr, hipEvent_t ev_stop = nullptr, uint32_t sub_log2 = 0);
 void launch_flush(hipStream_t st, u64 *atom, float4 *out, uint32_t *hot, uint32_t nbins, bool use_hot);
-void launch_clear_frame(hipStream_t st, float4 *front, u64 *atom, uint32_t *hot, u64 *counters, float4 *points,
-                        uint32_t nbins, uint32_t npoints);
+void launch_clear_frame(hipStream_t st, float4 *front, u64 *atom, uint32_t *hot, uint32_t nbins);
+void launch_clear_shared(hipStream_t st, u64 *counters, float4 *points, uint32_t npoints);
 void launch_shuffle_tap(hipStream_t st, int nw, uint32_t *out, uint32_t round);
 void launch_apply_xf_tap(hipStream_t st, const int32_t *prog, const float *params, uint32_t ts, int xfi,
                          uint32_t n, float4 *pts, fl_mwc *rng);
@@ -71,7 +71,8 @@
 
 struct DeTail { int do_log; float k1, k2; int do_clip; float vib, highpow, gam, lin, lingam; int order; };
 void launch_de_dir(hipStream_t st, fl_dim d, int pattern, float4 *Nout, const float4 *N, const float *coefs7,
-                   float sstd, float cstd, float dstd, float dpow, float gspeed, int in_mode = 1, const DeTail *tail = nullptr);
+                   float sstd, float cstd, float dstd, float dpow, float gspeed, int in_mode = 1, const DeTail *tail = nullptr,
+                   const u64 *cells = nullptr);
 
 void launch_de_adaptive(hipStream_t st, fl_dim d, float4 *buf, float4 *stage_c, float *stage_a, uint32_t *tmax,
                         const float *sinv, float R, float Rmin, float curve);
```

Measured after the change: 208,900 Msamples/s, median of 6. Within noise of the previous version (+0.4%).
